# blyssprivacy/sdk

Measured on AMD Instinct MI355X. Metric: PIR queries/sec (full answer path) on 2^20 items x 256 B, higher is better.
Workload: dtype u64; 1 GPU; spiral-rs process_query, c2 = {"db_item_size": 256, "instances": 1, "n": 2, "nu_1": 9, "nu_2": 11, "p": 256, "q2_bits": 20, "t_conv": 4, "t_exp_left": 8, "t_exp_right": 56, "t_gsw": 8}, encoded DB 64.0 GiB (56.0 GiB resident per GPU), unsharded, one query per step

## Files before the change

sdk_amd/csrc/bodies.hpp:

```cpp
#pragma once
#include "device_common.hpp"

namespace spiral {

__device__ __forceinline__ void ntt_fwd_body(const DevTables& T, const FwdDesc& d, int o, int c, u32* ldsA, u32* ldsB) {
  const int tau = threadIdx.x;
  const int rows = d.rdim * d.t;
  const int per_b = rows * d.cols;
  const int b = o / per_b;
  const int rem = o - b * per_b;
  const int row = rem / d.cols, col = rem - row * d.cols;
  const int kdig = row / d.rdim, j = row - kdig * d.rdim;
  long sb = d.src_idx ? (long)d.src_idx[b] : (long)b;
  if (d.delta_off) sb = (long)(b / d.delta_inner) * d.delta_outer_stride + (b % d.delta_inner);
  const u64* src = d.src + (sb * d.src_batch_stride + (long)(d.src_row0 + j) * d.src_cols + col) * N;
  const ModConst m = T.c.mod[c];
  const int sh = kdig * d.bits;
  const bool plain = (d.bits >= 64);
  const u64 mask = plain ? ~0ULL : ((1ULL << d.bits) - 1ULL);
  u32 v[8];
#pragma unroll
  for (int k = 0; k < 8; k++) {
    u64 x = src[tau + 256 * k];
    u64 piece = (sh >= 64) ? 0ULL : ((x >> sh) & mask);
    u32 val = (d.bits <= 28) ? (u32)piece : reduce64(piece, m);
    if (d.delta_off) {
      u64 x2 = src[(size_t)d.delta_off * N + tau + 256 * k];
      u64 piece2 = (sh >= 64) ? 0ULL : ((x2 >> sh) & mask);
      u32 val2 = (d.bits <= 28) ? (u32)piece2 : reduce64(piece2, m);
      u32 a = val >= m.q ? val - m.q : val, b2 = val2 >= m.q ? val2 - m.q : val2;
      val = b2 >= a ? b2 - a : b2 + m.q - a;
    }
    v[k] = val;
  }
  const u32* fw = T.tw + (size_t)c * 4 * N;
  ntt_fwd_block(v, tau, ldsA, ldsB, fw, fw + N, m.q, m.two_q);
  uint4* dst = reinterpret_cast<uint4*>(d.dst + ((size_t)o * 2 + c) * N + 8 * tau);
  dst[0] = make_uint4(v[0], v[1], v[2], v[3]);
  dst[1] = make_uint4(v[4], v[5], v[6], v[7]);
}

__device__ __forceinline__ void ntt_inv_body(const DevTables& T, const InvDesc& d, int blk, u32* ldsA, u32* ldsB) {
  const int tau = threadIdx.x;
  int p = blk;
  long base;
  long crt_stride = d.crt_stride, z_stride = d.z_stride;
  if (d.sweep_np > 0) {
    const long np = d.sweep_np;
    if ((np % 16) == 0 && ((long)d.n_polys % 128) == 0) {
      const int b = blk;
      const int xcd = b & 7, slot = b >> 3;
      const int grp = (slot >> 4) * 8 + xcd, within = slot & 15;
      const int groups_per_plane = (int)(np / 16) * 2;
      const int plane_g = grp / groups_per_plane, rem_g = grp % groups_per_plane;
      const int r_g = rem_g / (int)(np / 16), iig = rem_g % (int)(np / 16);
      p = (int)(((long)plane_g * np + iig * 16 + within) * 2 + r_g);
    }
    const long ct = p >> 1, r = p & 1;
    const long plane = ct / np, ii = ct - plane * np;
    base = plane * 4 * N * np + r * 2 * N * np + ii;
    crt_stride = N * np;
    z_stride = np;
  } else if (d.idx) {
    int e = p / d.polys_per_idx, r = p - e * d.polys_per_idx;
    base = (long)d.idx[e] * d.idx_stride + (long)r * d.poly_stride;
  } else {
    base = (long)p * d.poly_stride;
  }
  long scal_store = -1;
  if (d.scal) {
    if (p >= d.n_polys) {
      const int e = p - d.n_polys;
      const int ct = d.scal_only_idx[e >> 1], r = e & 1;
      const long sp = ((long)(ct - d.scal_thresh) * 2 + r) * 2 * N, dp = ((long)ct * 2 + r) * 2 * N;
#pragma unroll
      for (int c = 0; c < 2; c++) {
        const uint4* a = reinterpret_cast<const uint4*>(d.src + sp + c * N + 8 * tau);
        const uint4* b = reinterpret_cast<const uint4*>(d.scal + c * N + 8 * tau);
        const uint4 a0 = a[0], a1 = a[1], b0 = b[0], b1 = b[1];
        const ModConst m = T.c.mod[c];
        uint4* o = reinterpret_cast<uint4*>(d.scal_dst + dp + c * N + 8 * tau);
        o[0] = make_uint4(reduce64((u64)a0.x * b0.x, m), reduce64((u64)a0.y * b0.y, m), reduce64((u64)a0.z * b0.z, m), reduce64((u64)a0.w * b0.w, m));
        o[1] = make_uint4(reduce64((u64)a1.x * b1.x, m), reduce64((u64)a1.y * b1.y, m), reduce64((u64)a1.z * b1.z, m), reduce64((u64)a1.w * b1.w, m));
      }
      return;
    }
    const int e = p / d.polys_per_idx, r = p - e * d.polys_per_idx;
    const int ct = d.idx[e];
    if (ct >= d.scal_thresh) {
      scal_store = base;
      base = (long)(ct - d.scal_thresh) * d.idx_stride + (long)r * d.poly_stride;
    }
  }
  u32 res[2][8];
#pragma unroll
  for (int c = 0; c < 2; c++) {
    const ModConst m = T.c.mod[c];
    const u32* src = d.src + base + (long)c * crt_stride;
    u32 v[8];
    if (z_stride == 1 && ((base | crt_stride | (scal_store < 0 ? 0 : scal_store)) & 3) == 0) {
      const uint4 a0 = reinterpret_cast<const uint4*>(src + 8 * tau)[0], a1 = reinterpret_cast<const uint4*>(src + 8 * tau)[1];
      v[0] = a0.x; v[1] = a0.y; v[2] = a0.z; v[3] = a0.w; v[4] = a1.x; v[5] = a1.y; v[6] = a1.z; v[7] = a1.w;
      if (d.premod) {
#pragma unroll
        for (int k = 0; k < 8; k++) v[k] %= m.q;
      }
      if (scal_store >= 0) {
        const uint4 s0 = reinterpret_cast<const uint4*>(d.scal + c * N + 8 * tau)[0], s1 = reinterpret_cast<const uint4*>(d.scal + c * N + 8 * tau)[1];
        const u32 sc[8] = {s0.x, s0.y, s0.z, s0.w, s1.x, s1.y, s1.z, s1.w};
#pragma unroll
        for (int k = 0; k < 8; k++) v[k] = reduce64((u64)v[k] * (u64)sc[k], m);
        uint4* o = reinterpret_cast<uint4*>(d.scal_dst + scal_store + (long)c * crt_stride + 8 * tau);
        o[0] = make_uint4(v[0], v[1], v[2], v[3]);
        o[1] = make_uint4(v[4], v[5], v[6], v[7]);
      }
    } else {
#pragma unroll
      for (int k = 0; k < 8; k++) {
        u32 x = src[(long)(8 * tau + k) * z_stride];
        if (d.premod) x = x % m.q;
        if (scal_store >= 0) {
          x = reduce64((u64)x * (u64)d.scal[c * N + 8 * tau + k], m);
          d.scal_dst[scal_store + (long)c * crt_stride + 8 * tau + k] = x;
        }
        v[k] = x;
      }
    }
    const u32* iw = inv_tables(T.tw, c);
    if (c == 1) __syncthreads();
    ntt_inv_block(v, tau, ldsA, ldsB, iw, iw + N, m.q, m.two_q);
#pragma unroll
    for (int k = 0; k < 8; k++) res[c][k] = v[k];
  }
  const u32 q0 = T.c.mod[0].q, q1 = T.c.mod[1].q;
  u64* dst = d.dst + (size_t)p * N;
#pragma unroll
  for (int k = 0; k < 8; k++) {
    u32 x = res[0][k], y = res[1][k];
    u32 xm = x >= q1 ? x - q1 : x;
    u32 dd = y >= xm ? y - xm : y + q1 - xm;
    u32 qt = __umulhi(dd, T.c.q0_inv_q1_sh);
    u32 e = dd * T.c.q0_inv_q1 - qt * q1;
    e = e >= q1 ? e - q1 : e;
    u64 val = (u64)x + (u64)q0 * (u64)e;
    int z = tau + 256 * k;
    if (d.automorph_t) {
      unsigned zt = (unsigned)z * (unsigned)d.automorph_t;
      unsigned num = zt >> POLY_LEN_LOG2, rem = zt & (N - 1);
      dst[rem] = (num & 1u) ? T.c.Q - val : val;
    } else if (d.addend) {
      const long ap = (long)(p / d.add_inner2) * d.add_outer_stride + (p % d.add_inner2);
      u64 sres = val + d.addend[(size_t)ap * N + z];
      dst[z] = sres >= T.c.Q ? sres - T.c.Q : sres;
    } else {
      dst[z] = val;
    }
  }
}

template <int CH = 28>
__device__ __forceinline__ void mac_body(const DevTables& T, const MacDesc& d, int inner, int outer, int ychunk) {
  const int e = ychunk * 256 + threadIdx.x;
  const int c = e >> POLY_LEN_LOG2;
  const int b = outer * d.batch_inner + inner;
  const ModConst m = T.c.mod[c];
  const u32* B = d.B + ((size_t)outer * d.B_outer_stride + (size_t)inner * d.B_inner_stride) * 2 * N + e;
  const long ob = d.out_idx ? (long)d.out_idx[b] : (long)b * d.out_batch_stride;
  const size_t PW = 2 * N;
  for (int r = 0; r < d.R; r++) {
    const u32* A = d.A + (size_t)r * (d.A_row_stride ? d.A_row_stride : d.K) * PW + e;
    const long op = (ob + (long)r * d.out_row_stride) * 2 * N + e;
    u64 acc = d.addend ? (u64)d.addend[op] : 0ULL;
    if (d.extra && r == d.extra_row) acc += (u64)d.extra[(size_t)(d.extra_idx ? d.extra_idx[b] : b) * PW + e];
    for (int seg = 0; seg < 2; seg++) {
      const int k_lo = seg == 0 ? 0 : d.split_k, k_hi = seg == 0 ? min(d.split_k, d.K) : d.K;
      const u32* Bs = seg == 0 ? B : B + (size_t)(d.split_off - d.split_k) * PW;
      int k = k_lo, since = 0;
      for (; k + CH <= k_hi; k += CH) {
        u32 a[CH], bb[CH];
#pragma unroll
        for (int u = 0; u < CH; u++) {
          a[u] = A[(size_t)(k + u) * PW];
          bb[u] = Bs[(size_t)(k + u) * PW];
        }
#pragma unroll
        for (int u = 0; u < CH; u++) acc += (u64)a[u] * (u64)bb[u];
        since += CH;
        if (since >= 56) {
          acc = reduce64(acc, m);
          since = 0;
        }
      }
      for (; k + 8 <= k_hi; k += 8) {
        u32 a[8], bb[8];
#pragma unroll
        for (int u = 0; u < 8; u++) {
          a[u] = A[(size_t)(k + u) * PW];
          bb[u] = Bs[(size_t)(k + u) * PW];
        }
#pragma unroll
        for (int u = 0; u < 8; u++) acc += (u64)a[u] * (u64)bb[u];
        since += 8;
        if (since >= 64) {
          acc = reduce64(acc, m);
          since = 0;
        }
      }
      for (; k < k_hi; k++) acc += (u64)A[(size_t)k * PW] * (u64)Bs[(size_t)k * PW];
      acc = reduce64(acc, m);
    }
    d.out[op] = (u32)acc;
  }
}

__device__ __forceinline__ void add_poly_into_body(const DevTables& T, u32* dst, const int* idx, const u32* src, int b, int ychunk) {
  const int e = ychunk * 256 + threadIdx.x;
  const int c = e >> POLY_LEN_LOG2;
  const long dp = (long)idx[b] * 2 * N + e;
  dst[dp] = add_mod(dst[dp], src[(size_t)b * 2 * N + e], T.c.mod[c].q);
}

__device__ __forceinline__ void copy_polys_body(const CopyPolysDesc& d, int bx, int ychunk) {
  const int e = ychunk * 256 + threadIdx.x;
  const int b = bx / d.R, r = bx % d.R;
  d.dst[((long)d.dst_idx[b] + (long)r * d.dst_row_stride) * 2 * N + e] =
      d.src[((long)d.src_idx[b] + (long)r * d.src_row_stride) * 2 * N + e];
}

__device__ __forceinline__ void folding_neg_body(const DevTables& T, const FoldingNegDesc& d, int ychunk, int by, int dd) {
  const int e = ychunk * 256 + threadIdx.x;
  const int c = e >> POLY_LEN_LOG2;
  const int col = by % d.two_t, r = by / d.two_t;
  const u32 q = T.c.mod[c].q;
  u32* row = d.mats + ((size_t)(dd * 2 + r) * 2 * d.two_t) * 2 * N;
  const u32 cv = row[(size_t)(d.two_t + col) * 2 * N + e];
  const u32 g = d.gadget_ntt[((size_t)r * d.two_t + col) * 2 * N + e];
  row[(size_t)col * 2 * N + e] = add_mod(g, cv ? q - cv : 0u, q);
}

__device__ __forceinline__ void reorient_body(const ReorientDesc& d, int bx, int by, u64* tile) {
  const int tx = threadIdx.x & 31, ty = threadIdx.x >> 5;
  const int j0 = bx * 32, z0 = by * 32;
#pragma unroll
  for (int r = 0; r < 2; r++)
#pragma unroll
    for (int i = 0; i < 4; i++) {
      const int j = j0 + ty + 8 * i;
      if (j < d.dim0) {
        const u32* p = d.v + ((size_t)(d.first + d.step * j) * 2 + r) * 2 * N;
        tile[r * (32 * 33) + (ty + 8 * i) * 33 + tx] = (u64)p[z0 + tx] | ((u64)p[N + z0 + tx] << 32);
      }
    }
  __syncthreads();
  const int w = threadIdx.x & 63, jl = w >> 1, r = w & 1, zr = threadIdx.x >> 6;
  if (j0 + jl < d.dim0) {
#pragma unroll
    for (int i = 0; i < 8; i++) {
      const int zl = zr + 4 * i;
      d.out[((size_t)(z0 + zl) * d.dim0 + j0 + jl) * 2 + r] = tile[r * (32 * 33) + jl * 33 + zl];
    }
  }
}

__host__ __device__ inline int wave_layout_word(int n) { return ((n & 31) >> 2) * 256 + (n >> 5) * 4 + (n & 3); }
__device__ __forceinline__ void mats_to_wave_body(const MatsToWaveDesc& d, size_t blk) {
  const size_t idx = blk * 256 + threadIdx.x;
  if (idx >= d.n_words) return;
  const size_t poly = idx >> POLY_LEN_LOG2;
  if (d.half_polys > 0 && (((poly >> 1) / (size_t)d.half_polys) & 1) == 0) return;
  const int n = (int)(idx & (N - 1));
  d.dst[poly * N + wave_layout_word(n)] = d.src[idx];
}

__device__ __forceinline__ u64 rescale_dev(u64 a, u64 Q, u64 out_mod) {
  u64 v = a % Q;
  const bool neg = v >= Q / 2;
  const u64 mag = neg ? Q - v : v;
  u64 lo = mag * out_mod, hi = __umul64hi(mag, out_mod);
  const u64 half = Q / 2;
  lo += half;
  hi += lo < half ? 1 : 0;
  u64 qd = (u64)(((double)hi * 18446744073709551616.0 + (double)lo) / (double)Q);
  for (int it = 0; it < 4; it++) {
    const u64 plo = qd * Q, phi = __umul64hi(qd, Q);
    const bool gt = phi > hi || (phi == hi && plo > lo);
    if (gt) {
      qd--;
      continue;
    }
    const u64 rlo = lo - plo, rhi = hi - phi - (lo < plo ? 1 : 0);
    if (rhi != 0 || rlo >= Q) {
      qd++;
      continue;
    }
    break;
  }
  const u64 base = (Q / out_mod) * out_mod + 2 * out_mod;
  const u64 r = neg ? (base - qd) % out_mod : (base + qd) % out_mod;
  return (r + out_mod) % out_mod;
}

__device__ __forceinline__ void encode_body(const EncodeDesc& d, int blk) {
  const int per_inst_first = d.n * N, per_inst_rest = d.n * d.n * N;
  const int per_inst = per_inst_first + per_inst_rest;
  const long i = (long)blk * 256 + threadIdx.x;
  if (i >= (long)d.instances * per_inst) return;
  const int inst = (int)(i / per_inst), k = (int)(i % per_inst);
  const u64* m = d.packed + (size_t)inst * (d.n + 1) * d.n * N;
  const size_t inst_bits = (size_t)per_inst_first * d.q2_bits + (size_t)per_inst_rest * d.q1_bits;
  u64 val;
  size_t bit;
  int nb;
  if (k < per_inst_first) {
    val = rescale_dev(m[k], d.Q, d.q2);
    nb = d.q2_bits;
    bit = (size_t)inst * inst_bits + (size_t)k * d.q2_bits;
  } else {
    const int kk = k - per_inst_first;
    val = rescale_dev(m[per_inst_first + kk], d.Q, d.q1);
    nb = d.q1_bits;
    bit = (size_t)inst * inst_bits + (size_t)per_inst_first * d.q2_bits + (size_t)kk * d.q1_bits;
  }
  val &= nb >= 64 ? ~0ULL : ((1ULL << nb) - 1ULL);
  const size_t w = bit >> 6;
  const int off = (int)(bit & 63);
  atomicOr(d.out + w, (unsigned long long)(val << off));
  if (off + nb > 64) atomicOr(d.out + w + 1, (unsigned long long)(val >> (64 - off)));
}

}
```

sdk_amd/csrc/elementwise.hip:

```cpp
#include "device_common.hpp"
#include "bodies.hpp"

namespace spiral {

__global__ __launch_bounds__(256) void k_mac(DevTables T, MacDesc d) { mac_body(T, d, blockIdx.x, blockIdx.z, blockIdx.y); }
__global__ __launch_bounds__(256) void k_mac2(DevTables T, MacDesc d0, MacDesc d1) {
  const int y = blockIdx.x;
  if (y < d0.batch_inner)
    mac_body(T, d0, y, 0, blockIdx.y);
  else
    mac_body(T, d1, y - d0.batch_inner, 0, blockIdx.y);
}
__global__ __launch_bounds__(256) void k_mac2_group(DevTables T, MacDesc d0, MacDesc d1, GroupOff g) {
  const int qi = blockIdx.z;
  int y = blockIdx.x;
  MacDesc d = d0;
  if (y >= d0.batch_inner) {
    d = d1;
    y -= d0.batch_inner;
  }
  d.A = group_rebase(d.A, g.pp[qi]);
  d.B = group_rebase(d.B, g.dig[qi]);
  d.out = group_rebase(d.out, g.v[qi]);
  d.addend = group_rebase(d.addend, g.v[qi]);
  d.extra = group_rebase(d.extra, g.ct1[qi]);
  mac_body(T, d, y, 0, blockIdx.y);
}
void launch_mac2_group(const DevTables& T, const MacDesc& d0, const MacDesc& d1, const GroupOff& g, int B, hipStream_t s) {
  MacDesc a = d0, b = d1;
  a.batch_inner = std::max(a.batch_inner, 0);
  b.batch_inner = std::max(b.batch_inner, 0);
  if (a.batch_inner + b.batch_inner <= 0 || B <= 0) return;
  hipLaunchKernelGGL(k_mac2_group, dim3(a.batch_inner + b.batch_inner, 2 * N / 256, B), dim3(256), 0, s, T, a, b, g);
  launched(PATH_EXPAND_GROUP, "k_mac2_group");
}
void launch_mac(const DevTables& T, const MacDesc& d, hipStream_t s) {
  if (d.batch_inner <= 0 || d.batch_outer <= 0) return;
  hipLaunchKernelGGL(k_mac, dim3(d.batch_inner, 2 * N / 256, d.batch_outer), dim3(256), 0, s, T, d);
  launched(0, "k_mac");
}
void launch_mac2(const DevTables& T, const MacDesc& d0, const MacDesc& d1, hipStream_t s) {
  MacDesc a = d0, b = d1;
  a.batch_inner = std::max(a.batch_inner, 0);
  b.batch_inner = std::max(b.batch_inner, 0);
  if (a.batch_inner + b.batch_inner <= 0) return;
  hipLaunchKernelGGL(k_mac2, dim3(a.batch_inner + b.batch_inner, 2 * N / 256, 1), dim3(256), 0, s, T, a, b);
  launched(0, "k_mac2");
}

__global__ __launch_bounds__(256) void k_add_poly_into(DevTables T, u32* dst, const int* idx, const u32* src) {
  add_poly_into_body(T, dst, idx, src, blockIdx.x, blockIdx.y);
}
void launch_add_poly_into(const DevTables& T, u32* dst, const int* idx, const u32* src, int batch, hipStream_t s) {
  if (batch <= 0) return;
  hipLaunchKernelGGL(k_add_poly_into, dim3(batch, 2 * N / 256), dim3(256), 0, s, T, dst, idx, src);
  launched(0, "k_add_poly_into");
}

__global__ __launch_bounds__(256) void k_scalar_mul(DevTables T, u32* base, long dst_off, long src_off,
                                                    const u32* scalar) {
  const int e = blockIdx.y * 256 + threadIdx.x;
  const int c = e >> POLY_LEN_LOG2;
  const long b = blockIdx.x;
  const ModConst m = T.c.mod[c];
  base[(dst_off + b) * 2 * N + e] = reduce64((u64)base[(src_off + b) * 2 * N + e] * (u64)scalar[e], m);
}
void launch_scalar_mul(const DevTables& T, u32* base, long dst_off, long src_off, const u32* scalar, int n_polys,
                       hipStream_t s) {
  if (n_polys <= 0) return;
  hipLaunchKernelGGL(k_scalar_mul, dim3(n_polys, 2 * N / 256), dim3(256), 0, s, T, base, dst_off, src_off, scalar);
  launched(0, "k_scalar_mul");
}

__global__ __launch_bounds__(256) void k_add_polys_idx(DevTables T, u32* dst, const int* di, const u32* a, const int* ai,
                                                        const u32* b, const int* bi) {
  const int e = blockIdx.y * 256 + threadIdx.x;
  const int c = e >> POLY_LEN_LOG2;
  const int k = blockIdx.x;
  dst[(size_t)di[k] * 2 * N + e] = add_mod(a[(size_t)ai[k] * 2 * N + e], b[(size_t)bi[k] * 2 * N + e], T.c.mod[c].q);
}
void launch_add_polys_idx(const DevTables& T, u32* dst, const int* di, const u32* a, const int* ai, const u32* b,
                          const int* bi, int count, hipStream_t s) {
  if (count <= 0) return;
  hipLaunchKernelGGL(k_add_polys_idx, dim3(count, 2 * N / 256), dim3(256), 0, s, T, dst, di, a, ai, b, bi);
  launched(0, "k_add_polys_idx");
}

__global__ __launch_bounds__(256) void k_interleave_query(u64* qv, const u32* row0_ntt, const u64* wire, int dim0, u32 q0,
                                                          u32 q1) {
  const size_t i = (size_t)blockIdx.x * 256 + threadIdx.x;
  if (i >= (size_t)N * dim0) return;
  const int j = (int)(i % dim0);
  const int z = (int)(i / dim0);
  const u32* p = row0_ntt + (size_t)j * 2 * N;
  qv[2 * i] = (u64)p[z] | ((u64)p[N + z] << 32);
  const u64 w = wire[i];
  qv[2 * i + 1] = (u64)((u32)w % q0) | ((u64)((u32)(w >> 32) % q1) << 32);
}
void launch_interleave_query(u64* qv, const u32* row0_ntt, const u64* wire, int dim0, hipStream_t s) {
  size_t total = (size_t)N * dim0;
  hipLaunchKernelGGL(k_interleave_query, dim3((unsigned)((total + 255) / 256)), dim3(256), 0, s, qv, row0_ntt, wire, dim0,
                     (u32)MODULUS_0, (u32)MODULUS_1);
  launched(0, "k_interleave_query");
}

__global__ __launch_bounds__(256) void k_copy_polys(CopyPolysDesc d) { copy_polys_body(d, blockIdx.x, blockIdx.y); }
void launch_copy_polys(u32* dst, const int* dst_idx, int dst_row_stride, const u32* src, const int* src_idx,
                       int src_row_stride, int R, int batch, hipStream_t s) {
  if (batch <= 0) return;
  const CopyPolysDesc d{dst, dst_idx, dst_row_stride, src, src_idx, src_row_stride, R, batch};
  hipLaunchKernelGGL(k_copy_polys, dim3(batch * R, 2 * N / 256), dim3(256), 0, s, d);
  launched(0, "k_copy_polys");
}

__global__ __launch_bounds__(256) void k_copy_polys_group(CopyPolysDesc d, GroupOff g) {
  const int qi = blockIdx.z;
  d.dst = group_rebase(d.dst, g.raw[qi]);
  d.src = group_rebase(d.src, g.v[qi]);
  copy_polys_body(d, blockIdx.x, blockIdx.y);
}
void launch_copy_polys_group(u32* dst, const int* dst_idx, int dst_row_stride, const u32* src, const int* src_idx, int src_row_stride,
                             int R, int batch, const GroupOff& g, int B, hipStream_t s) {
  if (batch <= 0 || B <= 0) return;
  const CopyPolysDesc d{dst, dst_idx, dst_row_stride, src, src_idx, src_row_stride, R, batch};
  hipLaunchKernelGGL(k_copy_polys_group, dim3(batch * R, 2 * N / 256, B), dim3(256), 0, s, d, g);
  launched(PATH_EXPAND_GROUP, "k_copy_polys_group");
}

__global__ __launch_bounds__(256) void k_checksum(const u32* p, size_t n, unsigned long long* out) {
  unsigned long long acc = 0;
  for (size_t i = (size_t)blockIdx.x * 256 + threadIdx.x; i < n; i += (size_t)gridDim.x * 256)
    acc += (unsigned long long)p[i] * (unsigned long long)((i << 1) | 1);
  atomicAdd(out, acc);
}
void launch_checksum(const u32* p, size_t n_words, unsigned long long* out, hipStream_t s) {
  hipLaunchKernelGGL(k_checksum, dim3(512), dim3(256), 0, s, p, n_words, out);
  launched(0, "k_checksum");
}
__global__ __launch_bounds__(64) void k_cache_sync(u32* sink) {
  __threadfence_system();
  if (sink && threadIdx.x == 0 && blockIdx.x == 0) sink[0] = 1;
  __threadfence_system();
}
void launch_cache_sync(u32* sink, hipStream_t s) {
  hipLaunchKernelGGL(k_cache_sync, dim3(1024), dim3(64), 0, s, sink);
  launched(0, "k_cache_sync");
}

__global__ __launch_bounds__(256) void k_copy_words(u32* dst, const u32* src, size_t n) {
  for (size_t i = (size_t)blockIdx.x * 256 + threadIdx.x; i < n; i += (size_t)gridDim.x * 256) dst[i] = src[i];
}
void launch_copy_words(u32* dst, const u32* src, size_t n_words, hipStream_t s) {
  if (n_words == 0) return;
  const unsigned blocks = (unsigned)std::min<size_t>((n_words + 255) / 256, 4096);
  hipLaunchKernelGGL(k_copy_words, dim3(blocks), dim3(256), 0, s, dst, src, n_words);
  launched(0, "k_copy_words");
}

__global__ __launch_bounds__(256) void k_folding_neg(DevTables T, FoldingNegDesc d) {
  folding_neg_body(T, d, blockIdx.x, blockIdx.y, blockIdx.z);
}
void launch_folding_neg(const DevTables& T, u32* mats, const u32* gadget_ntt, int nu2, int two_t, hipStream_t s) {
  if (nu2 <= 0) return;
  const FoldingNegDesc d{mats, gadget_ntt, two_t, nu2};
  hipLaunchKernelGGL(k_folding_neg, dim3(2 * N / 256, 2 * two_t, nu2), dim3(256), 0, s, T, d);
  launched(0, "k_folding_neg");
}

__global__ __launch_bounds__(256) void k_folding_neg_group(DevTables T, FoldingNegDesc d, GroupOff g) {
  const int qi = blockIdx.z / d.nu2;
  d.mats = group_rebase(d.mats, g.v[qi]);
  folding_neg_body(T, d, blockIdx.x, blockIdx.y, blockIdx.z - qi * d.nu2);
}
void launch_folding_neg_group(const DevTables& T, u32* mats, const u32* gadget_ntt, int nu2, int two_t, const GroupOff& g, int B,
                              hipStream_t s) {
  if (nu2 <= 0 || B <= 0) return;
  const FoldingNegDesc d{mats, gadget_ntt, two_t, nu2};
  hipLaunchKernelGGL(k_folding_neg_group, dim3(2 * N / 256, 2 * two_t, nu2 * B), dim3(256), 0, s, T, d, g);
  launched(PATH_EXPAND_GROUP, "k_folding_neg_group");
}

__global__ __launch_bounds__(256) void k_add(DevTables T, u32* out, const u32* a, const u32* b) {
  const size_t i = (size_t)blockIdx.x * 256 + threadIdx.x;
  const int c = (int)((i >> POLY_LEN_LOG2) & 1);
  out[i] = add_mod(a[i], b[i], T.c.mod[c].q);
}
void launch_add(const DevTables& T, u32* out, const u32* a, const u32* b, int n_polys, hipStream_t s) {
  if (n_polys <= 0) return;
  hipLaunchKernelGGL(k_add, dim3((unsigned)((size_t)n_polys * 2 * N / 256)), dim3(256), 0, s, T, out, a, b);
  launched(0, "k_add");
}

__global__ __launch_bounds__(256) void k_invert_raw(u64 Q, u64* out, const u64* a, long n) {
  long i = (long)blockIdx.x * 256 + threadIdx.x;
  if (i < n) out[i] = Q - a[i];
}
void launch_invert_raw(const DevTables& T, u64* out, const u64* a, long n_words, hipStream_t s) {
  if (n_words <= 0) return;
  hipLaunchKernelGGL(k_invert_raw, dim3((unsigned)((n_words + 255) / 256)), dim3(256), 0, s, T.c.Q, out, a, n_words);
  launched(0, "k_invert_raw");
}

__global__ __launch_bounds__(256) void k_automorph(u64 Q, u64* out, const u64* a, int t) {
  const int z = blockIdx.y * 256 + threadIdx.x;
  const size_t p = (size_t)blockIdx.x * N;
  unsigned zt = (unsigned)z * (unsigned)t;
  unsigned num = zt >> POLY_LEN_LOG2, rem = zt & (N - 1);
  u64 v = a[p + z];
  out[p + rem] = (num & 1u) ? Q - v : v;
}
void launch_automorph(const DevTables& T, u64* out, const u64* a, int n_polys, int t, hipStream_t s) {
  if (n_polys <= 0) return;
  hipLaunchKernelGGL(k_automorph, dim3(n_polys, N / 256), dim3(256), 0, s, T.c.Q, out, a, t);
  launched(0, "k_automorph");
}

__global__ __launch_bounds__(256) void k_gadget_raw(u64* out, const u64* inp, int cols, int rdim, int bits) {
  const int z = blockIdx.y * 256 + threadIdx.x;
  const int o = blockIdx.x;
  const int row = o / cols, col = o - row * cols;
  const int k = row / rdim, j = row - k * rdim;
  const int sh = k * bits;
  const u64 mask = bits >= 64 ? ~0ULL : ((1ULL << bits) - 1ULL);
  u64 x = inp[((size_t)j * cols + col) * N + z];
  out[(size_t)o * N + z] = sh >= 64 ? 0ULL : ((x >> sh) & mask);
}
void launch_gadget_raw(u64* out, const u64* inp, int rows_in, int cols, int rows_out, int rdim, int bits,
                       hipStream_t s) {
  (void)rows_in;
  hipLaunchKernelGGL(k_gadget_raw, dim3(rows_out * cols, N / 256), dim3(256), 0, s, out, inp, cols, rdim, bits);
  launched(0, "k_gadget_raw");
}

__global__ __launch_bounds__(256) void k_u64_to_u32(u32* out, const u64* in, long n) {
  long i = (long)blockIdx.x * 256 + threadIdx.x;
  if (i < n) out[i] = (u32)in[i];
}
__global__ __launch_bounds__(256) void k_u32_to_u64(u64* out, const u32* in, long n) {
  long i = (long)blockIdx.x * 256 + threadIdx.x;
  if (i < n) out[i] = (u64)in[i];
}
void launch_u64_to_u32(u32* out, const u64* in, long n, hipStream_t s) {
  if (n <= 0) return;
  hipLaunchKernelGGL(k_u64_to_u32, dim3((unsigned)((n + 255) / 256)), dim3(256), 0, s, out, in, n);
  launched(0, "k_u64_to_u32");
}
void launch_u32_to_u64(u64* out, const u32* in, long n, hipStream_t s) {
  if (n <= 0) return;
  hipLaunchKernelGGL(k_u32_to_u64, dim3((unsigned)((n + 255) / 256)), dim3(256), 0, s, out, in, n);
  launched(0, "k_u32_to_u64");
}

__global__ __launch_bounds__(256) void k_encode(EncodeDesc d) { encode_body(d, blockIdx.x); }
void launch_encode(const EncodeDesc& d, hipStream_t s) {
  const long total = (long)d.instances * ((long)d.n * N + (long)d.n * d.n * N);
  hipLaunchKernelGGL(k_encode, dim3((unsigned)((total + 255) / 256)), dim3(256), 0, s, d);
  launched(0, "k_encode");
}

__global__ __launch_bounds__(256) void k_reorient(ReorientDesc d) {
  __shared__ u64 tile[2 * 32 * 33];
  reorient_body(d, blockIdx.x, blockIdx.y, tile);
}
void launch_reorient(u64* out, const u32* v, int first, int step, int dim0, hipStream_t s) {
  const ReorientDesc d{out, v, first, step, dim0};
  hipLaunchKernelGGL(k_reorient, dim3((dim0 + 31) / 32, N / 32), dim3(256), 0, s, d);
  launched(0, "k_reorient");
}

__global__ __launch_bounds__(256) void k_reorient_group(ReorientDesc d, GroupOff g) {
  __shared__ u64 tile[2 * 32 * 33];
  const int qi = blockIdx.z;
  d.out = group_rebase(d.out, g.raw[qi]);
  d.v = group_rebase(d.v, g.v[qi]);
  reorient_body(d, blockIdx.x, blockIdx.y, tile);
}
void launch_reorient_group(u64* out, const u32* v, int first, int step, int dim0, const GroupOff& g, int B, hipStream_t s) {
  if (B <= 0) return;
  const ReorientDesc d{out, v, first, step, dim0};
  hipLaunchKernelGGL(k_reorient_group, dim3((dim0 + 31) / 32, N / 32, B), dim3(256), 0, s, d, g);
  launched(PATH_EXPAND_GROUP, "k_reorient_group");
}

__global__ __launch_bounds__(64) void k_cu_probe(u32* out) {
  u32 xcc, hw;
  asm volatile("s_getreg_b32 %0, hwreg(HW_REG_XCC_ID)" : "=s"(xcc));
  asm volatile("s_getreg_b32 %0, hwreg(HW_REG_HW_ID)" : "=s"(hw));
  u32 acc = threadIdx.x;
  for (int i = 0; i < 20000; i++) acc = acc * 1664525u + 1013904223u;
  if (threadIdx.x == 0) {
    out[blockIdx.x * 2] = xcc;
    out[blockIdx.x * 2 + 1] = hw | ((acc & 1u) << 31);
  }
}
void launch_cu_probe(u32* out, int blocks, hipStream_t s) {
  hipLaunchKernelGGL(k_cu_probe, dim3(blocks), dim3(64), 0, s, out);
  launched(0, "k_cu_probe");
}

}

#include "pp_raw_image.hpp"
```

sdk_amd/csrc/kernels.hpp:

```cpp
#pragma once
#include <hip/hip_runtime.h>

#include <vector>

#include "params.hpp"

namespace spiral {

constexpr int N = (int)POLY_LEN;

struct DevTables {
  const u32* tw;
  DevConsts c;
};
__host__ __device__ inline const u32* inv_tables(const u32* tw, int c) { return tw + (size_t)8 * N + (size_t)c * 2 * N; }
__host__ __device__ inline const u32* wave_fwd_image(const u32* tw, int c) { return tw + (size_t)12 * N + (size_t)c * 2 * N; }
__host__ __device__ inline int wtw_phys(int idx) {
  if (idx >= 1024) {
    const int L = (idx - 1024) >> 4, r = (idx - 1024) & 15;
    return 1024 + 16 * L + 4 * (((r >> 2) + (L >> 2)) & 3) + (r & 3);
  }
  if (idx >= 512) {
    const int L = (idx - 512) >> 3, r = (idx - 512) & 7;
    return 512 + 8 * L + 4 * (((r >> 2) + (L >> 3)) & 1) + (r & 3);
  }
  return idx;
}

enum PathBit : u64 {
  PATH_SWEEP_PERSIST = 1ull << 0,
  PATH_SWEEP_PACKED = 1ull << 1,
  PATH_SWEEP_WIDE = 1ull << 2,
  PATH_SWEEP_NARROW = 1ull << 3,
  PATH_SWEEP_BATCH = 1ull << 4,
  PATH_FROM_SWEEP4 = 1ull << 5,
  PATH_FROM_SWEEP1 = 1ull << 6,
  PATH_FOLD_FUSED = 1ull << 7,
  PATH_FOLD_TAIL = 1ull << 8,
  PATH_FOLD_TAIL_LITERAL = 1ull << 9,
  PATH_PIPELINED = 1ull << 10,
  PATH_EXPAND_PRUNED = 1ull << 11,
  PATH_PACK_V1 = 1ull << 12,
  PATH_DIRECT_UPLOAD = 1ull << 13,
  PATH_SCATTER_OUT = 1ull << 14,
  PATH_SWEEP_XCD_FROM = 1ull << 15,
  PATH_FOLD_TAIL_PERSIST = 1ull << 16,
  PATH_EXPAND_FUSED = 1ull << 17,
  PATH_SWEEP_SPARSE = 1ull << 18,
  PATH_RCCL = 1ull << 19,
  PATH_FOLD_WAVE = 1ull << 20,
  PATH_CU_SPLIT = 1ull << 21,
  PATH_EXPAND_SPLIT = 1ull << 22,
  PATH_PIPE_CLASS_SPLIT = 1ull << 23,
  PATH_SWEEP_MFMA = 1ull << 24,
  PATH_CUSTOM_TRANSPORT = 1ull << 25,
  PATH_FROM_SWEEP_WAVE = 1ull << 26,
  PATH_FOLD_TAIL_BATCHED = 1ull << 27,
  PATH_SWEEP_RING = 1ull << 28,
  PATH_SWEEP_MFMA2 = 1ull << 29,
  PATH_FOLD_WAVE8 = 1ull << 30,
  PATH_SWEEP_PLANAR = 1ull << 31,
  PATH_EXPAND_GROUP = 1ull << 32,
  PATH_EXPAND_WAVE = 1ull << 33,
  PATH_SWEEP_BATCH_SCATTER = 1ull << 34,
  PATH_SWEEP_SPARSE_GROUP = 1ull << 35,
  PATH_SWEEP_NARROW_GROUP = 1ull << 36
};
long tunable(const char* name, long dflt);
void launched(u64 path_bits, const char* kernel);
void note_path(u64 path_bits);
void launch_checksum(const u32* p, size_t n_words, unsigned long long* out, hipStream_t s);
void launch_cache_sync(u32* sink, hipStream_t s);
void launch_copy_words(u32* dst, const u32* src, size_t n_words, hipStream_t s);
void debug_stage(int stage);

struct FwdDesc {
  const u64* src;
  const int* src_idx;
  u32* dst;
  int n_out;
  int rdim, cols, t, bits;
  int src_batch_stride;
  int src_row0, src_cols;
  long delta_off;
  int delta_inner, delta_outer_stride;
};
void launch_ntt_fwd(const DevTables& T, const FwdDesc& d, hipStream_t s);
void launch_ntt_fwd3(const DevTables& T, const FwdDesc& d0, const FwdDesc& d1, const FwdDesc& d2, hipStream_t s);

float bench_ntt_core(const DevTables& T, int M, int blocks, int reps, u32* scratch, hipStream_t s);

struct InvDesc {
  const u32* src;
  const int* idx;
  int polys_per_idx;
  long idx_stride, poly_stride, crt_stride, z_stride;
  u64* dst;
  int n_polys;
  int premod;
  int sweep_np;
  int automorph_t;
  const u32* scal;
  u32* scal_dst;
  int scal_thresh;
  const int* scal_only_idx;
  int n_scalar_only;
  const u64* addend;
  int add_inner2, add_outer_stride;
};
void launch_ntt_inv(const DevTables& T, const InvDesc& d, hipStream_t s);
void launch_from_sweep4(const DevTables& T, const u32* src, int np, int n_planes, int premod, u64* dst, hipStream_t s);

struct MacDesc {
  const u32* A;
  const u32* B;
  u32* out;
  const u32* addend;
  const int* out_idx;
  int R, K;
  int A_row_stride;
  int batch_inner, batch_outer;
  long B_inner_stride, B_outer_stride;
  int split_k;
  long split_off;
  int out_batch_stride, out_row_stride;
  const u32* extra;
  const int* extra_idx;
  int extra_row;
};
void launch_mac(const DevTables& T, const MacDesc& d, hipStream_t s);
void launch_mac2(const DevTables& T, const MacDesc& d0, const MacDesc& d1, hipStream_t s);

struct ExpandSideDesc {
  const u64* raw;
  const int* pos;
  const int* out_idx;
  const u32* A;
  u32* v;
  int cnt, t, bits;
};
void launch_expand_round(const DevTables& T, const ExpandSideDesc& left, const ExpandSideDesc& right, hipStream_t s);
constexpr long EXPAND_ROUND_MIN_DEFAULT = 2048;

constexpr int GROUP_MAX = 16;
struct GroupOff {
  long long v[GROUP_MAX], raw[GROUP_MAX], dig[GROUP_MAX], ct1[GROUP_MAX], pp[GROUP_MAX];
};
void launch_ntt_inv_group(const DevTables& T, const InvDesc& d, const GroupOff& g, int B, hipStream_t s);
void launch_ntt_fwd3_group(const DevTables& T, const FwdDesc& d0, const FwdDesc& d1, const FwdDesc& d2, const GroupOff& g, int B,
                           hipStream_t s);
void launch_mac2_group(const DevTables& T, const MacDesc& d0, const MacDesc& d1, const GroupOff& g, int B, hipStream_t s);
void launch_expand_round_group(const DevTables& T, const ExpandSideDesc& left, const ExpandSideDesc& right, const GroupOff& g, int B,
                               hipStream_t s);
void launch_reorient_group(u64* out, const u32* v, int first, int step, int dim0, const GroupOff& g, int B, hipStream_t s);
void launch_copy_polys_group(u32* dst, const int* dst_idx, int dst_row_stride, const u32* src, const int* src_idx, int src_row_stride,
                             int R, int batch, const GroupOff& g, int B, hipStream_t s);
void launch_folding_neg_group(const DevTables& T, u32* mats, const u32* gadget_ntt, int nu2, int two_t, const GroupOff& g, int B,
                              hipStream_t s);
void launch_mats_to_wave_group(u32* dst, const u32* src, size_t n_words, int half_polys, const GroupOff& g, int B, hipStream_t s);
struct ExpandWaveDesc {
  const u64* raw;
  const int* pos;
  const int* out_idx;
  const u32* A_w;
  const u32* const_w;
  u32* v;
  int cnt, t, bits;
};
void launch_expand_wave(const DevTables& T, const ExpandWaveDesc& d, const GroupOff& g, int B, hipStream_t s);
constexpr long EXPAND_WAVE_MIN_DIGITS_DEFAULT = 16;
constexpr long EXPAND_GROUP_ROUND_MIN_DEFAULT = 4096;

struct FoldDesc {
  const u64* X;
  u64* Y;
  const u32* mats;
  int cur, half, planes;
  int t, bits;
  int t_live;
  int zero_shortcuts;
  const u32* mats_w;
};
void launch_mats_to_wave(u32* dst, const u32* src, size_t n_words, hipStream_t s, int half_polys = 0);
constexpr long FOLD_VARIANT_DEFAULT = 5;
void launch_fold_fused(const DevTables& T, const FoldDesc& d, hipStream_t s);

void launch_add_poly_into(const DevTables& T, u32* dst, const int* idx, const u32* src, int batch, hipStream_t s);
void launch_scalar_mul(const DevTables& T, u32* base, long dst_off, long src_off, const u32* scalar, int n_polys,
                       hipStream_t s);
void launch_add_polys_idx(const DevTables& T, u32* dst, const int* di, const u32* a, const int* ai, const u32* b,
                          const int* bi, int count, hipStream_t s);
void launch_interleave_query(u64* qv, const u32* row0_ntt, const u64* wire, int dim0, hipStream_t s);
void launch_copy_polys(u32* dst, const int* dst_idx, int dst_row_stride, const u32* src, const int* src_idx,
                       int src_row_stride, int R, int batch, hipStream_t s);
void launch_folding_neg(const DevTables& T, u32* mats, const u32* gadget_ntt, int nu2, int two_t, hipStream_t s);
void launch_add(const DevTables& T, u32* out, const u32* a, const u32* b, int n_polys, hipStream_t s);
void launch_invert_raw(const DevTables& T, u64* out, const u64* a, long n_words, hipStream_t s);
void launch_automorph(const DevTables& T, u64* out, const u64* a, int n_polys, int t, hipStream_t s);
void launch_gadget_raw(u64* out, const u64* inp, int rows_in, int cols, int rows_out, int rdim, int bits,
                       hipStream_t s);
void launch_u64_to_u32(u32* out, const u64* in, long n, hipStream_t s);
void launch_u32_to_u64(u64* out, const u32* in, long n, hipStream_t s);

void launch_cu_probe(u32* out, int blocks, hipStream_t s);

struct EncodeDesc {
  const u64* packed;
  unsigned long long* out;
  int instances, n;
  u64 Q, q1, q2;
  int q1_bits, q2_bits;
};
void launch_encode(const EncodeDesc& d, hipStream_t s);

void launch_reorient(u64* out, const u32* v, int first, int step, int dim0, hipStream_t s);

struct CopyPolysDesc {
  u32* dst;
  const int* dst_idx;
  int dst_row_stride;
  const u32* src;
  const int* src_idx;
  int src_row_stride, R, batch;
};
struct FoldingNegDesc {
  u32* mats;
  const u32* gadget_ntt;
  int two_t, nu2;
};
struct ReorientDesc {
  u64* out;
  const u32* v;
  int first, step, dim0;
};
struct MatsToWaveDesc {
  u32* dst;
  const u32* src;
  size_t n_words;
  int half_polys;
};
struct AddPolyIntoDesc {
  u32* dst;
  const int* idx;
  const u32* src;
  int batch;
};
struct CopyWordsDesc {
  u32* dst;
  const u32* src;
  size_t n_words;
};
constexpr u64 PP_RAW_WIRE = 1ull << 63;
struct PpRawDesc {
  u64* dst;
  const u64* wire;
  const u64* table;
  u64 n_words;
  u64 modulus, modulus_inv;
};
void launch_pp_raw_image(const PpRawDesc& d, int n_polys, hipStream_t s);

struct SweepDesc {
  const u64* db;
  const u64* qv;
  u32* out;
  int planes, num_per, dim0, j0, nj;
  int packed;
  int out_G;
  int nt_store;
};
struct ColMap {
  int off = 0, stride = 1, np_global = 0;
};
inline bool db_can_pack(int num_per, int nj) { return num_per >= 128 && (nj % 2) == 0; }
inline size_t db_bytes(int planes, int num_per, int nj, bool packed) {
  return (size_t)planes * N * nj * num_per * (packed ? 7 : 8);
}
void launch_sweep(const DevTables& T, const SweepDesc& d, hipStream_t s);
void launch_sweep_persist(const DevTables& T, const SweepDesc& d, int wgs_per_cu, hipStream_t s, int n_cus = 256);
constexpr int SWEEP_BATCH_MAX = 8;
constexpr int SWEEP_GROUP_MAX = 16;
struct SweepBatchDesc {
  const u64* db;
  const u64* qv[SWEEP_GROUP_MAX];
  u32* out[SWEEP_GROUP_MAX];
  int batch;
  int planes, num_per, dim0, j0, nj;
  u32* rq;
  int use_mfma;
  const unsigned char* planar;
  int narrow;
  int fold_every;
};
bool sweep_narrow_batch_shape_ok(int num_per, int nj);
constexpr long NARROW_BATCH_MIN_DEFAULT = 0;
void launch_sweep_narrow_batch(const DevTables& T, const SweepBatchDesc& d, hipStream_t s);
bool sweep_planar_shape_ok(int num_per, int nj);
size_t sweep_planar_bytes(int planes, int num_per, int nj);
void launch_packed_to_planar(unsigned char* planar, const u64* packed, int planes, int num_per, int nj, hipStream_t s);
void launch_planar_patch_item(unsigned char* planar, const u64* packed, int planes, int num_per, int nj, int j, int ii, hipStream_t s);
constexpr size_t UPSERT_MAX_GROUP_PLANES = (size_t)1 << 23;
struct PlanarPatchCell {
  int j, ii;
};
void launch_planar_patch_items(unsigned char* planar, const u64* packed, int planes, int num_per, int nj, const PlanarPatchCell* cells,
                               size_t n_cells, hipStream_t s);
void launch_sweep_planar(const DevTables& T, const SweepBatchDesc& d, hipStream_t s);
bool planar_resident_shape_ok(int num_per, int nj);
int planar_resident_group_max(int nj);
struct PlanarShardShape {
  int dim0 = 0;
  int j0 = 0;
  int G = 1;
};
void launch_planar_from_ref(unsigned char* planar, const u64* src, int plane, int z0, int nz, int num_per, int nj, PlanarShardShape sh,
                            hipStream_t s);
void launch_planar_synth(unsigned char* planar, u64 seed, int planes, int num_per, int nj, PlanarShardShape sh, hipStream_t s);
void launch_planar_from_stage(unsigned char* planar, const u64* stage, int planes, int jg, int ii0, int ncols, int num_per, int nj,
                              PlanarShardShape sh, hipStream_t s);
void launch_planar_put_items(unsigned char* planar, const u64* stage, int planes, size_t np_s, const PlanarPatchCell* cells, size_t n_items,
                             int num_per, int nj, PlanarShardShape sh, hipStream_t s);
void launch_planar_read(u64* out, const unsigned char* planar, int plane, int z, int ii, int jl0, int count, int num_per, int nj,
                        PlanarShardShape sh, hipStream_t s);
void sweep_planar_resident_prepare(const DevTables& T, SweepBatchDesc& d, hipStream_t s);
void launch_sweep_planar_resident(const DevTables& T, const SweepBatchDesc& d, hipStream_t s);
void launch_sweep_planar_scatter(const DevTables& T, const SweepBatchDesc& d, int G, int plane0, int total_planes, bool all_planes,
                                 hipStream_t s);
bool sweep_batch_wants_mfma(const SweepBatchDesc& d);
int sweep_batch_group_max(int num_per, int nj);
inline int sweep_batch_tiles(int batch) { return batch > SWEEP_BATCH_MAX ? 2 : 1; }
inline size_t sweep_batch_rq_words(int nj, int tiles = 1) {
  return (size_t)tiles * ((size_t)N * (size_t)(nj / 16) * 128 * 4 + (size_t)N * 32);
}
void sweep_batch_prepare(const DevTables& T, SweepBatchDesc& d, hipStream_t s);
void launch_sweep_batch(const DevTables& T, const SweepBatchDesc& d, hipStream_t s);
constexpr long BATCH_SCATTER_STORE_DEFAULT = 2;
constexpr long BATCH_SCATTER_MAX_G_DEFAULT = 8;
bool sweep_batch_scatter_ok(const SweepBatchDesc& d, int G);
void launch_sweep_batch_scatter(const DevTables& T, const SweepBatchDesc& d, int G, hipStream_t s);
void launch_db_relayout(u64* dst, int plane, const u64* src, int z0, int nz, int num_per, int dim0, int j0, int nj,
                        int packed, ColMap cm, hipStream_t s);
void launch_canon_words(u64* w, size_t total, hipStream_t s);
void launch_db_synth(u64* dst, u64 seed, int planes, int num_per, int dim0, int j0, int nj, int packed, ColMap cm,
                     hipStream_t s);
void launch_db_read(u64* out, const u64* db, int plane, int z, int ii, int jl0, int count, int num_per, int nj,
                    int packed, hipStream_t s);
struct DbEncodeDesc {
  const uint8_t* win;
  size_t win_item0;
  size_t win_bytes;
  size_t file_len;
  u64* db;
  int db_item_size, bytes_per_chunk, logp;
  u32 pt_modulus;
  int planes, num_per, dim0, j0, nj, packed;
  int jp0, njp;
  long only_item;
  int only_q;
  ColMap cm;
};
void launch_db_encode(const DevTables& T, const DbEncodeDesc& d, hipStream_t s);
struct DbQuadRec {
  int jp, q;
  int len[4];
  long long src[4];
};
void launch_db_encode_quads(const DevTables& T, const DbEncodeDesc& d, const DbQuadRec* quads, size_t n_quads, hipStream_t s);

void launch_items_gather(u64* dst, const u64* db, size_t L0, size_t nL, int np_local, int nj, int planes, int packed, hipStream_t s);
void launch_planar_gather(u64* dst, const unsigned char* planar, size_t L0, size_t nL, int num_per, int nj, int planes, PlanarShardShape sh,
                          hipStream_t s);
struct ItemDecodeRec {
  int src, pos;
};
struct ItemDecodeDesc {
  const u64* src;
  const ItemDecodeRec* list;
  uint8_t* out;
  unsigned long long* undecodable;
  int planes, db_item_size, bytes_per_chunk, logp;
  u32 pt_modulus;
};
void launch_items_decode(const DevTables& T, const ItemDecodeDesc& d, size_t n_items, hipStream_t s);

void launch_items_scatter_words8(u64* db, const u64* stage, const int* src_of, size_t D0, size_t nD, int np_local, int nj, int planes,
                                 hipStream_t s);
struct CopyQuadRec {
  int jp, q;
  int src[4];
};
void launch_items_scatter_packed(u64* db, const u64* stage, const CopyQuadRec* quads, size_t n_quads, int np_local, int nj, int planes,
                                 hipStream_t s);
struct CopyCellRec {
  int j, ii;
  int src[16];
};
void launch_planar_scatter_items(unsigned char* planar, const u64* stage, const CopyCellRec* cells, size_t n_cells, int num_per, int nj,
                                 int planes, PlanarShardShape sh, hipStream_t s);
struct CopySlotRec {
  int src, slot;
};
void launch_items_copy_slots(u64* polys, const u64* stage, const CopySlotRec* recs, size_t n_recs, int planes, hipStream_t s);

void launch_sparse_item_encode(const DevTables& T, const uint8_t* bytes, int item_bytes, int bytes_per_chunk, int logp,
                               u32 pt_modulus, u64* slot_polys, int planes, hipStream_t s);
struct SparseItemRec {
  unsigned long long off;
  int len, slot;
};
void launch_sparse_items_encode(const DevTables& T, const uint8_t* win, const SparseItemRec* items, size_t n_items, int item_bytes,
                                int bytes_per_chunk, int logp, u32 pt_modulus, u64* polys, int planes, hipStream_t s);
void launch_sweep_sparse(const DevTables& T, const int* col_ptr, const int* col_rows, const int* col_slots, const u64* polys,
                         int planes, const u32* v, int first, int step, u32* out, int num_per, hipStream_t s);
constexpr int SPARSE_GROUP_MAX = 8;
constexpr long SPARSE_BATCH_MIN_DEFAULT = 2;
struct SparseGroup {
  const u32* v[SPARSE_GROUP_MAX];
  u32* out[SPARSE_GROUP_MAX];
};
void launch_sweep_sparse_batch(const DevTables& T, const int* col_ptr, const int* col_rows, const int* col_slots, const u64* polys,
                               int planes, const SparseGroup& members, int nq, int first, int step, int num_per, hipStream_t s);
void launch_sweep_sparse_scatter(const DevTables& T, const int* col_ptr, const int* col_rows, const int* col_slots, const u64* polys,
                                 int planes, int plane0, int n_planes, const u32* v, int first, int step, u32* out, int num_per, int G,
                                 bool per_plane, hipStream_t s);
void launch_sweep_sparse_scatter_batch(const DevTables& T, const int* col_ptr, const int* col_rows, const int* col_slots, const u64* polys,
                                       int planes, const SparseGroup& members, int nq, int first, int step, int num_per, int G,
                                       hipStream_t s);

void launch_sweep_out_to_ref(u64* out, const u32* in, int num_per, hipStream_t s);

__host__ __device__ inline u64 synth_word(u64 seed, u64 idx) {
  u64 z = seed + 0x9E3779B97F4A7C15ULL * (idx + 1);
  z = (z ^ (z >> 30)) * 0xBF58476D1CE4E5B9ULL;
  z = (z ^ (z >> 27)) * 0x94D049BB133111EBULL;
  z ^= z >> 31;
  u64 lo = (u32)z % (u32)MODULUS_0;
  u64 hi = (u32)(z >> 32) % (u32)MODULUS_1;
  return lo | (hi << 32);
}

__host__ __device__ inline u64 digest_mix(u64 x) {
  x += 0x9E3779B97F4A7C15ULL;
  x = (x ^ (x >> 30)) * 0xBF58476D1CE4E5B9ULL;
  x = (x ^ (x >> 27)) * 0x94D049BB133111EBULL;
  return x ^ (x >> 31);
}
__host__ __device__ inline u64 digest_col_key(u64 s, u64 c) { return digest_mix(s ^ c) | 1ULL; }
__host__ __device__ inline u64 digest_row_key(u64 s, u64 j) { return digest_mix(~s ^ j) | 1ULL; }
constexpr int DIGEST_ROWS = 1024;
struct DigestDesc {
  unsigned long long* sums;
  const u64* R;
  u64 s[2];
  int plane0, nplanes;
  int num_per;
  int nj;
};
void launch_digest_keys(unsigned long long* sums, u64* R, u64 seed, int nplanes, int j0, int nj, hipStream_t s);
void launch_digest_words(const DigestDesc& d, const u64* db, int np_local, int packed, ColMap cm, hipStream_t s);
struct DigestSlotRec {
  unsigned long long slot, item;
};
void launch_digest_sparse(const DigestDesc& d, const u64* polys, int planes, const DigestSlotRec* list, size_t n, hipStream_t s);
void launch_digest_planar(const DigestDesc& d, const unsigned char* planar, PlanarShardShape sh, hipStream_t s);

constexpr int ITEM_DIGEST_Z = 64;
struct ItemDigestDesc {
  unsigned long long* table;
  const u64* R;
  u64 s[2];
  int plane0, nplanes;
  int num_per;
  int nj;
  int jl0, nrows;
};
void launch_item_digest_words(const ItemDigestDesc& d, const u64* db, int np_local, int packed, ColMap cm, hipStream_t s);
void launch_item_digest_sparse(const ItemDigestDesc& d, const u64* polys, int planes, const DigestSlotRec* list, size_t n,
                               unsigned long long item_base, uint8_t* present, hipStream_t s);
void launch_item_digest_planar(const ItemDigestDesc& d, const unsigned char* planar, PlanarShardShape sh, hipStream_t s);

}
```

sdk_amd/csrc/pipeline.hpp:

```cpp
#pragma once
#include <vector>

#include "server.hpp"

namespace spiral {

struct Workspace {
  const Params* P;
  DeviceState* D;
  int device = -1;
  hipStream_t stream = nullptr;
  hipStream_t stream2 = nullptr;
  std::vector<hipEvent_t> ev_plane;
  hipEvent_t ev_fold = nullptr;
  hipEvent_t ev_round0 = nullptr, ev_right = nullptr;
  bool right_pending = false;
  bool long_sweep_follows = false;
  hipEvent_t ev_sw[2] = {nullptr, nullptr};
  bool have_sweep_span = false;
  bool pipelined = false;
  hipEvent_t ev[5] = {nullptr, nullptr, nullptr, nullptr, nullptr};
  DevBuf<u64> q_raw;
  DevBuf<u32> v;
  DevBuf<u64> exp_raw;
  DevBuf<u32> exp_dig;
  DevBuf<u32> exp_ct1;
  DevBuf<u64> exp_raw_r;
  DevBuf<u32> exp_dig_r, exp_ct1_r;
  DevBuf<u64> qv;
  DevBuf<u32> fold_mats;
  DevBuf<u32> fold_mats_w;
  bool mats_w_ready = false;
  DevBuf<u64> gsw_raw;
  DevBuf<u32> gsw_dig;
  DevBuf<u32> sweep_out;
  DevBuf<u64> fold_tail;
  DevBuf<u32> batch_rq;
  DevBuf<u64> foldX, foldY, final_cts, pack_raw;
  DevBuf<u32> fold_dig, fold_ntt, pack_dig, pack_ct2, pack_res, pack_v1_P, pack_v1_P2;
  DevBuf<u64> pack_v1_raw, du_raw, du_wire;
  DevBuf<u32> du_ntt;
  u64* h_query = nullptr;
  u64* h_group_query = nullptr;
  DevBuf<u64> group_q_raw;
  u64* h_packed = nullptr;
  size_t h_packed_words = 0;
  DevBuf<u64> enc_out;
  uint8_t* h_response = nullptr;
  bool host_pinned = true;
  int out_G = 1;
  bool zero_shortcuts = false;
  long fused_min_pairs = 256;

  Workspace(const Params& P, DeviceState& D);
  ~Workspace();
  Workspace(const Workspace&) = delete;
  Workspace& operator=(const Workspace&) = delete;
  void ensure_expand();
  void ensure_sweep();
  void ensure_finish();
  size_t plane_group() const;
};

void run_coefficient_expansion(Workspace& W, const sp_pp& pp, size_t g_rounds, const DeviceState::PrunedPlan* plan = nullptr,
                               int tree = 0, size_t r_begin = 0);
void join_right(Workspace& W);
void run_regev_to_gsw(Workspace& W, const sp_pp& pp, const u32* v_src, const int* src_ct, const int* src_poly);
void run_folding_neg(Workspace& W);
void run_mats_to_wave(Workspace& W, size_t levels, bool c_only = false);
void run_fold_operands(Workspace& W);
void run_begin_direct(Workspace& W, const uint8_t* query);
void run_begin_group(Workspace* const* Ws, const sp_pp* const* pps, const uint8_t* const* queries, const size_t* query_lens, int B);
void run_begin(Workspace& W, const sp_pp& pp, const uint8_t* query, size_t query_len, int j0 = 0, int nj = 0,
               const DeviceState::PrunedPlan* plan = nullptr);
void run_sweep_sparse(Workspace& W, const sp_db& db, const int* col_ptr, const int* col_rows, const int* col_slots);
void run_sweep_sparse_group(Workspace* const* Ws, int B, const sp_db& db, const int* col_ptr, const int* col_rows, const int* col_slots,
                            hipStream_t s);
void run_sweep_sparse_scatter(Workspace& W, const sp_db& db, const int* col_ptr, const int* col_rows, const int* col_slots, int G,
                              int plane0, int n_planes, bool per_plane);
void run_sweep_sparse_scatter_group(Workspace* const* Ws, int B, const sp_db& db, const int* col_ptr, const int* col_rows,
                                    const int* col_slots, int G, hipStream_t s);
std::unique_ptr<DeviceState::PrunedPlan> build_pruned_plan_rows(const Params& P, const std::vector<char>& rows);
void run_sweep(Workspace& W, const sp_db& db);
void run_sweep_pipelined(Workspace& W, const sp_db& db);
bool sweep_is_pipelined(const Params& p, const sp_db& db);
void launch_plane_sweep(Workspace& W, const sp_db& db, size_t plane);
bool fused_fold_supported(const Params& p);
struct FoldOpts {
  long fused_min_pairs;
  bool delta_tail;
  bool inputs_below_q;
};
u64* run_fold(Workspace& W, const FoldOpts& o, u64* X, u64* Y, int np, int num_cts, int top, int d_begin = 0, int d_end = -1);
void run_fold_local(Workspace& W, const u32* reduced_chunk, int G);
void run_fold_local_plane(Workspace& W, const u32* reduced_plane_chunk, int G, int plane);
void run_fold_local_join(Workspace& W);
void run_finish_gathered(Workspace& W, const sp_pp& pp, const u64* gathered, int G);
void run_fold_all(Workspace& W, bool premod);
void run_pack(Workspace& W, const sp_pp& pp);
void run_finish(Workspace& W, const sp_pp& pp, bool premod);
size_t encode_response(const Params& p, const u64* packed, uint8_t* out);
void run_encode_device(Workspace& W);

}
```

sdk_amd/csrc/server.cpp:

```cpp
#include "server.hpp"

#include <algorithm>
#include <atomic>
#include <cstdlib>
#include <cstring>
#include <functional>

#include "pipeline.hpp"

namespace spiral {

void hip_check(hipError_t e, const char* what, const char* file, int line) {
  if (e != hipSuccess) {
    (void)hipGetLastError();
    throw HipError(std::string(what) + " failed at " + file + ":" + std::to_string(line) + ": " + hipGetErrorString(e));
  }
}

static std::mutex g_tun_mu;
static std::vector<std::pair<std::string, long>> g_tun;
static std::atomic<unsigned> g_tun_epoch{1};
static std::atomic<long> g_fresh_allocs{0};
void tunables_new_call() { g_tun_epoch.fetch_add(1, std::memory_order_relaxed); }
void set_tunable(const char* name, long v) {
  if (!strcmp(name, "poison_skip")) g_fresh_allocs = 0;
  {
    std::lock_guard<std::mutex> lk(g_tun_mu);
    bool found = false;
    for (auto& kv : g_tun)
      if (kv.first == name) {
        kv.second = v;
        found = true;
        break;
      }
    if (!found) g_tun.emplace_back(name, v);
  }
  tunables_new_call();
}
static bool tunable_resolve(const char* name, long* out) {
  {
    std::lock_guard<std::mutex> lk(g_tun_mu);
    for (auto& kv : g_tun)
      if (kv.first == name) {
        *out = kv.second;
        return true;
      }
  }
  std::string env = "SPIRAL_";
  for (const char* c = name; *c; c++) env += (char)toupper((unsigned char)*c);
  const char* e = getenv(env.c_str());
  if (!e) return false;
  *out = atol(e);
  return true;
}
long tunable(const char* name, long dflt) {
  struct Ent {
    std::string name;
    unsigned epoch;
    bool has;
    long val;
  };
  thread_local std::vector<Ent> cache;
  const unsigned ep = g_tun_epoch.load(std::memory_order_relaxed);
  for (auto& e : cache)
    if (!strcmp(e.name.c_str(), name)) {
      if (e.epoch != ep) {
        e.has = tunable_resolve(name, &e.val);
        e.epoch = ep;
      }
      return e.has ? e.val : dflt;
    }
  Ent e{name, ep, false, 0};
  e.has = tunable_resolve(name, &e.val);
  cache.push_back(e);
  return e.has ? e.val : dflt;
}

void devbuf_fresh(void* p, size_t bytes) {
  const long b = tunable("poison_ws", 0);
  if (b <= 0 || !p || tunable("guard_ws", 0) > 0) return;
  const long k = g_fresh_allocs.fetch_add(1);
  const bool skip = tunable("poison_skip", -1) == k;
  if (getenv("SPIRAL_ALLOC_DEBUG")) fprintf(stderr, "[spiral] alloc #%ld: %zu bytes%s\n", k, bytes, skip ? " (zeroed)" : "");
  HIP_CHECK(hipMemset(p, skip ? 0 : (int)(b & 255), bytes));
  HIP_CHECK(hipDeviceSynchronize());
}
void devbuf_cache_sync();
bool devbuf_guards_on() { return tunable("guard_ws", 0) > 0; }
void* devbuf_alloc(size_t bytes, size_t* guard, long* serial) {
  const long g = tunable("guard_ws", 0);
  const size_t gb = g > 0 ? ((size_t)g + 255) / 256 * 256 : 0;
  void* q = nullptr;
  const hipError_t e = hipMalloc(&q, bytes + 2 * gb);
  if (e != hipSuccess) {
    (void)hipGetLastError();
    throw OomError(std::string("hipMalloc of ") + std::to_string(bytes) + " bytes failed: " + hipGetErrorString(e));
  }
  *guard = gb;
  *serial = -1;
  if (getenv("SPIRAL_ALLOC_DEBUG")) fprintf(stderr, "[spiral] hipMalloc %zu bytes -> [%p, %p)\n", bytes + 2 * gb, q, (char*)q + bytes + 2 * gb);
  void* const block = q;
  try {
  if (gb) {
    const long k = g_fresh_allocs.fetch_add(1);
    *serial = k;
    const bool skip = tunable("poison_skip", -1) == k;
    const int fill = skip ? 0 : (int)(tunable("poison_ws", 0xA5) & 255);
    if (getenv("SPIRAL_ALLOC_DEBUG")) fprintf(stderr, "[spiral] alloc #%ld: %zu bytes%s\n", k, bytes, skip ? " (guards zeroed)" : "");
    HIP_CHECK(hipMemset(q, fill, gb));
    HIP_CHECK(hipMemset((char*)q + gb + bytes, fill, gb));
    HIP_CHECK(hipDeviceSynchronize());
    q = (char*)q + gb;
  }
  devbuf_fresh(q, bytes);
  if (!gb && tunable("poison_ws", 0) <= 0 && tunable("alloc_zero", 1) != 0) {
    HIP_CHECK(hipMemset(q, 0, bytes));
    devbuf_cache_sync();
    HIP_CHECK(hipDeviceSynchronize());
  }
  } catch (...) {
    (void)hipFree(block);
    throw;
  }
  return q;
}
void devbuf_cache_sync() {
  if (tunable("alloc_cache_sync", 0) != 0) launch_cache_sync(nullptr, 0);
}
void devbuf_free(void* p, size_t bytes, size_t guard, long serial) {
  if (!p) return;
  if (getenv("SPIRAL_ALLOC_DEBUG")) fprintf(stderr, "[spiral] hipFree %p\n", (void*)((char*)p - guard));
  if (guard) {
    (void)hipDeviceSynchronize();
    std::vector<unsigned char> h(2 * guard);
    if (hipMemcpy(h.data(), (char*)p - guard, guard, hipMemcpyDeviceToHost) == hipSuccess &&
        hipMemcpy(h.data() + guard, (char*)p + bytes, guard, hipMemcpyDeviceToHost) == hipSuccess) {
      long first_before = -1, last_after = -1;
      for (size_t i = 0; i < guard; i++)
        if (h[i] != h[0]) { first_before = (long)(guard - i); break; }
      for (size_t i = 0; i < guard; i++)
        if (h[guard + i] != h[2 * guard - 1]) last_after = (long)i;
      if (first_before >= 0 || last_after >= 0)
        fprintf(stderr, "[spiral] OUT-OF-BOUNDS WRITE around alloc #%ld (%zu bytes): reaches %ld bytes before / %ld bytes after\n",
                serial, bytes, first_before, last_after);
    }
    (void)hipGetLastError();
  }
  (void)hipFree((char*)p - guard);
}

extern thread_local int g_debug_stage;
void h2d_sync(void* dst, const void* host, size_t bytes) {
  if (bytes == 0) return;
  HIP_CHECK(hipMemcpy(dst, host, bytes, hipMemcpyHostToDevice));
  if (tunable("h2d_cache_sync", 0) != 0) launch_cache_sync(nullptr, 0);
}
void upload_words(void* dst, const void* host, size_t bytes) {
  h2d_sync(dst, host, bytes);
  HIP_CHECK(hipDeviceSynchronize());
}

static thread_local u64 g_paths = 0;
void note_path(u64 bits) { g_paths |= bits; }
u64 paths_taken(bool reset) {
  const u64 v = g_paths;
  if (reset) g_paths = 0;
  return v;
}
void launched(u64 bits, const char* kernel) {
  g_paths |= bits;
  const hipError_t e = hipGetLastError();
  if (e != hipSuccess) throw HipError(std::string("launch of ") + kernel + " failed: " + hipGetErrorString(e));
  const long ds = tunable("debug_sync", 0);
  if (ds == 1 || (ds > 10 && ds == 10 + g_debug_stage)) HIP_CHECK(hipDeviceSynchronize());
}
thread_local int g_debug_stage = 0;
void debug_stage(int stage) {
  g_debug_stage = stage;
  if (tunable("debug_sync", 0) == 2) HIP_CHECK(hipDeviceSynchronize());
}

static inline u32 rotl(u32 v, int c) { return (v << c) | (v >> (32 - c)); }
static inline void quarter(u32* s, int a, int b, int c, int d) {
  s[a] += s[b]; s[d] = rotl(s[d] ^ s[a], 16);
  s[c] += s[d]; s[b] = rotl(s[b] ^ s[c], 12);
  s[a] += s[b]; s[d] = rotl(s[d] ^ s[a], 8);
  s[c] += s[d]; s[b] = rotl(s[b] ^ s[c], 7);
}
static void chacha_block(const u32 init[16], u64 ctr, u32 out[16]) {
  u32 in0[16], s[16];
  memcpy(in0, init, sizeof(in0));
  in0[12] = (u32)ctr;
  in0[13] = (u32)(ctr >> 32);
  in0[14] = in0[15] = 0;
  memcpy(s, in0, sizeof(s));
  for (int rnd = 0; rnd < 10; rnd++) {
    quarter(s, 0, 4, 8, 12); quarter(s, 1, 5, 9, 13); quarter(s, 2, 6, 10, 14); quarter(s, 3, 7, 11, 15);
    quarter(s, 0, 5, 10, 15); quarter(s, 1, 6, 11, 12); quarter(s, 2, 7, 8, 13); quarter(s, 3, 4, 9, 14);
  }
  for (int i = 0; i < 16; i++) out[i] = s[i] + in0[i];
}
#if defined(__x86_64__)
}
#include <immintrin.h>
namespace spiral {
__attribute__((target("avx2"))) static void chacha_blocks8_avx2(const u32 init[16], u64 ctr0, u32 (*out)[16]) {
  __m256i in0[16], s[16];
  for (int i = 0; i < 16; i++) in0[i] = _mm256_set1_epi32((int)init[i]);
  alignas(32) u32 lo[8], hi[8];
  for (int l = 0; l < 8; l++) {
    const u64 c = ctr0 + (u64)l;
    lo[l] = (u32)c;
    hi[l] = (u32)(c >> 32);
  }
  in0[12] = _mm256_load_si256(reinterpret_cast<const __m256i*>(lo));
  in0[13] = _mm256_load_si256(reinterpret_cast<const __m256i*>(hi));
  in0[14] = in0[15] = _mm256_setzero_si256();
  for (int i = 0; i < 16; i++) s[i] = in0[i];
#define SP_ROT(x, n) _mm256_or_si256(_mm256_slli_epi32(x, n), _mm256_srli_epi32(x, 32 - n))
#define SP_QR(a, b, c, d)                                                                              \
  s[a] = _mm256_add_epi32(s[a], s[b]); s[d] = _mm256_xor_si256(s[d], s[a]); s[d] = SP_ROT(s[d], 16);   \
  s[c] = _mm256_add_epi32(s[c], s[d]); s[b] = _mm256_xor_si256(s[b], s[c]); s[b] = SP_ROT(s[b], 12);   \
  s[a] = _mm256_add_epi32(s[a], s[b]); s[d] = _mm256_xor_si256(s[d], s[a]); s[d] = SP_ROT(s[d], 8);    \
  s[c] = _mm256_add_epi32(s[c], s[d]); s[b] = _mm256_xor_si256(s[b], s[c]); s[b] = SP_ROT(s[b], 7);
  for (int rnd = 0; rnd < 10; rnd++) {
    SP_QR(0, 4, 8, 12) SP_QR(1, 5, 9, 13) SP_QR(2, 6, 10, 14) SP_QR(3, 7, 11, 15)
    SP_QR(0, 5, 10, 15) SP_QR(1, 6, 11, 12) SP_QR(2, 7, 8, 13) SP_QR(3, 4, 9, 14)
  }
#undef SP_QR
#undef SP_ROT
  alignas(32) u32 tmp[16][8];
  for (int i = 0; i < 16; i++) _mm256_store_si256(reinterpret_cast<__m256i*>(tmp[i]), _mm256_add_epi32(s[i], in0[i]));
  for (int l = 0; l < 8; l++)
    for (int i = 0; i < 16; i++) out[l][i] = tmp[i][l];
}
static bool cpu_has_avx2() { return __builtin_cpu_supports("avx2"); }
#else
static void chacha_blocks8_avx2(const u32*, u64, u32 (*)[16]) {}
static bool cpu_has_avx2() { return false; }
#endif

void chacha20_keystream_u64(const uint8_t seed[32], u64* out, size_t count) {
  u32 init[16] = {0x61707865u, 0x3320646eu, 0x79622d32u, 0x6b206574u};
  for (int i = 0; i < 8; i++) {
    u32 w;
    memcpy(&w, seed + 4 * i, 4);
    init[4 + i] = w;
  }
  static const bool avx2 = cpu_has_avx2();
  const bool wide = avx2 && tunable("chacha_scalar", 0) == 0;
  u64 ctr = 0;
  size_t done = 0;
  u32 blk[8][16];
  while (done < count) {
    int have = 1;
    if (wide && count - done >= 16) {
      chacha_blocks8_avx2(init, ctr, blk);
      have = 8;
    } else {
      chacha_block(init, ctr, blk[0]);
    }
    ctr += (u64)have;
    for (int l = 0; l < have && done < count; l++)
      for (int i = 0; i < 16 && done < count; i += 2, done++) out[done] = (u64)blk[l][i] | ((u64)blk[l][i + 1] << 32);
  }
}

struct FastMod {
  u64 Q, m;
  explicit FastMod(u64 q) : Q(q), m(q > 1 ? (u64)(((unsigned __int128)1 << 64) / q) : 0) {}
  u64 operator()(u64 x) const {
    u64 r = x - (u64)(((unsigned __int128)x * m) >> 64) * Q;
    while (r >= Q) r -= Q;
    return r;
  }
};

static std::vector<RoundPlan> build_round_plans(const Params& P, int j0, int nj, std::vector<int>& L,
                                                const std::vector<char>* row_set = nullptr, int side = 0) {
  auto put = [&](const std::vector<int>& v) {
    size_t off = L.size();
    L.insert(L.end(), v.begin(), v.end());
    return off;
  };
  std::vector<RoundPlan> rounds;
  const size_t g = P.g();
  const size_t nu2 = P.db_dim_2;
  const size_t stop_round = nu2 > 0 ? P.stop_round() : 0;
  const size_t max_bits_right = nu2 > 0 ? P.t_gsw * nu2 : 0;
  const bool prune = nu2 > 0 && (row_set != nullptr || j0 != 0 || nj != (int)P.dim0());
  for (size_t r = 0; r < g; r++) {
    RoundPlan rp;
    rp.num_in = 1 << r;
    rp.t_auto = (int)(POLY_LEN >> r) + 1;
    std::vector<char> need_even((size_t)2 << r, 1);
    if (prune) {
      std::fill(need_even.begin(), need_even.end(), 0);
      const size_t mod = (size_t)2 << r;
      if (row_set) {
        for (size_t j = 0; j < row_set->size(); j++)
          if ((*row_set)[j]) need_even[((size_t)2 * j) % mod] = 1;
      } else if ((size_t)nj * 2 >= mod) {
        std::fill(need_even.begin(), need_even.end(), 1);
      } else {
        for (int j = j0; j < j0 + nj; j++) need_even[((size_t)2 * j) % mod] = 1;
      }
    }
    std::vector<int> all_ct, all_row1, lpos, lout, rpos, rout, skip2, lct, rct;
    for (int half = 0; half < 2; half++)
      for (int i = 0; i < rp.num_in; i++) {
        bool skip = (stop_round > 0 && r > stop_round && (i % 2) == 1) ||
                    (stop_round > 0 && r == stop_round && (i % 2) == 1 && (size_t)(i / 2) >= max_bits_right);
        const int ct = half * rp.num_in + i;
        const bool even_tree = r != 0 && (i % 2) == 0;
        if ((side == 1 && !even_tree) || (side == 2 && even_tree)) continue;
        if (skip) {
          if (half == 1 && !prune) skip2.push_back(rp.num_in + i);
          continue;
        }
        if (r != 0 && (i % 2) == 0 && !need_even[ct]) continue;
        int pos = (int)all_ct.size();
        all_ct.push_back(ct);
        all_row1.push_back(ct * 2 + 1);
        if (r != 0 && (i % 2) == 0) {
          lpos.push_back(pos);
          lout.push_back(ct * 2);
          lct.push_back(ct);
        } else {
          rpos.push_back(pos);
          rout.push_back(ct * 2);
          rct.push_back(ct);
        }
      }
    rp.n_all = (int)all_ct.size();
    rp.n_left = (int)lpos.size();
    rp.n_right = (int)rpos.size();
    rp.all_ct = put(all_ct);
    rp.all_row1 = put(all_row1);
    rp.left_pos = put(lpos);
    rp.left_out = put(lout);
    rp.right_pos = put(rpos);
    rp.right_out = put(rout);
    rp.left_ct = put(lct);
    rp.right_ct = put(rct);
    rp.skip2 = put(skip2);
    rp.n_skip2 = (int)skip2.size();
    rounds.push_back(rp);
  }
  return rounds;
}

const DeviceState::PrunedPlan& DeviceState::pruned_plan(const Params& P, int j0, int nj) {
  std::lock_guard<std::mutex> lk(pruned_mu);
  for (auto& pp : pruned)
    if (pp->j0 == j0 && pp->nj == nj) return *pp;
  auto pl = std::make_unique<PrunedPlan>();
  pl->j0 = j0;
  pl->nj = nj;
  std::vector<int> L;
  pl->rounds = build_round_plans(P, j0, nj, L);
  pl->rounds_even = build_round_plans(P, j0, nj, L, nullptr, 1);
  pl->rounds_odd = build_round_plans(P, j0, nj, L, nullptr, 2);
  pl->lists.alloc(std::max<size_t>(L.size(), 1));
  if (!L.empty()) upload_words(pl->lists.p, L.data(), L.size() * sizeof(int));
  pruned.push_back(std::move(pl));
  return *pruned.back();
}

std::unique_ptr<DeviceState::PrunedPlan> build_pruned_plan_rows(const Params& P, const std::vector<char>& rows) {
  auto pl = std::make_unique<DeviceState::PrunedPlan>();
  pl->j0 = -1;
  pl->nj = -1;
  std::vector<int> L;
  pl->rounds = build_round_plans(P, 0, 0, L, &rows);
  pl->rounds_even = build_round_plans(P, 0, 0, L, &rows, 1);
  pl->rounds_odd = build_round_plans(P, 0, 0, L, &rows, 2);
  pl->lists.alloc(std::max<size_t>(L.size(), 1));
  if (!L.empty()) upload_words(pl->lists.p, L.data(), L.size() * sizeof(int));
  return pl;
}

static std::unique_ptr<DeviceState> build_device_state(const Params& P, int device) {
  auto D = std::make_unique<DeviceState>();
  D->device = device;
  D->tw.alloc(P.ntt_tables.size());
  upload_words(D->tw.p, P.ntt_tables.data(), P.ntt_tables.size() * sizeof(u32));
  D->T.tw = D->tw.p;
  D->T.c = P.dc;
  const size_t g = P.expand_queries ? P.g() : 0;
  const size_t nu2 = P.db_dim_2;

  {
    std::vector<u64> raw(std::max<size_t>(g, 1) * POLY_LEN, 0);
    for (size_t r = 0; r < g && r < POLY_LEN_LOG2; r++) raw[r * POLY_LEN + (POLY_LEN - ((size_t)1 << r))] = P.modulus - 1;
    DevBuf<u64> d_raw(raw.size());
    h2d_sync(d_raw.p, raw.data(), raw.size() * 8);
    D->neg1.alloc(std::max<size_t>(g, 1) * 2 * POLY_LEN);
    FwdDesc f{d_raw.p, nullptr, D->neg1.p, (int)g, 1, 1, 1, 64, 1, 0, 1};
    launch_ntt_fwd(D->T, f, 0);
    HIP_CHECK(hipDeviceSynchronize());
  }
  {
    const size_t cols = 2 * P.t_gsw, bits = P.bits_per(P.t_gsw);
    std::vector<u64> raw(2 * cols * POLY_LEN, 0);
    for (size_t i = 0; i < 2; i++)
      for (size_t j = 0; j < P.t_gsw; j++) {
        if (bits * j >= 64) continue;
        raw[(i * cols + (i + j * 2)) * POLY_LEN] = 1ULL << (bits * j);
      }
    DevBuf<u64> d_raw(raw.size());
    h2d_sync(d_raw.p, raw.data(), raw.size() * 8);
    D->gadget_gsw.alloc(2 * cols * 2 * POLY_LEN);
    FwdDesc f{d_raw.p, nullptr, D->gadget_gsw.p, (int)(2 * cols), 1, 1, 1, 64, 1, 0, 1};
    launch_ntt_fwd(D->T, f, 0);
    HIP_CHECK(hipDeviceSynchronize());
  }

  std::vector<int> L;
  auto put = [&](const std::vector<int>& v) {
    size_t off = L.size();
    L.insert(L.end(), v.begin(), v.end());
    return off;
  };
  if (P.expand_queries) {
    D->rounds = build_round_plans(P, 0, (int)P.dim0(), L);
    D->rounds_even = build_round_plans(P, 0, (int)P.dim0(), L, nullptr, 1);
    D->rounds_odd = build_round_plans(P, 0, (int)P.dim0(), L, nullptr, 2);
    for (const RoundPlan& rp : D->rounds) {
      D->max_all = std::max(D->max_all, (size_t)rp.n_all);
      D->max_left = std::max(D->max_left, (size_t)rp.n_left);
      D->max_right = std::max(D->max_right, (size_t)rp.n_right);
    }
  }
  {
    std::vector<int> src_ct, src_poly, out_even, out_odd;
    for (size_t d = 0; d < nu2; d++)
      for (size_t j = 0; j < P.t_gsw; j++) {
        int b = (int)(d * P.t_gsw + j);
        src_ct.push_back(2 * b + 1);
        src_poly.push_back((2 * b + 1) * 2);
        int row0 = (int)(d * 2 * 4 * P.t_gsw + 2 * P.t_gsw);
        out_even.push_back(row0 + (int)(2 * j));
        out_odd.push_back(row0 + (int)(2 * j + 1));
      }
    D->gsw_src_ct = put(src_ct);
    D->gsw_src_poly = put(src_poly);
    D->gsw_out_even = put(out_even);
    D->gsw_out_odd = put(out_odd);
  }
  {
    std::vector<int> src_ct, out, row;
    const int n = (int)P.n;
    for (int inst = 0; inst < (int)P.instances; inst++)
      for (int c = 0; c < n; c++) {
        out.push_back(inst * (n + 1) * n + c);
        for (int r = 0; r < n; r++) {
          src_ct.push_back(inst * n * n + r * n + c);
          row.push_back(inst * (n + 1) * n + (1 + r) * n + c);
        }
      }
    D->pack_src_ct = put(src_ct);
    D->pack_out = put(out);
    D->pack_row = put(row);
  }
  if (P.version == 1 && P.n == 2) {
    std::vector<int> row1, ssrc, rd, ra, rb, sd, sa, sb;
    const int ne = (int)P.instances * 2;
    for (int b = 0; b < ne * 2; b++) row1.push_back(b * 3 + 1);
    for (int e = 0; e < ne; e++) {
      const int inst = e / 2, c = e % 2, b0 = e * 2, b1 = e * 2 + 1;
      ssrc.push_back(b1 * 3);
      rd.push_back(e * 3 + 1); ra.push_back(e * 3 + 1); rb.push_back(b1 * 3 + 2);
      rd.push_back(e * 3 + 2); ra.push_back(e * 3 + 2); rb.push_back(b1 * 3 + 1);
      for (int rr = 0; rr < 3; rr++) {
        sd.push_back(inst * 6 + rr * 2 + c);
        sa.push_back(b0 * 3 + rr);
        sb.push_back(e * 3 + rr);
      }
    }
    D->v1_row1 = put(row1);
    D->v1_shift_src = put(ssrc);
    D->v1_rot_dst = put(rd); D->v1_rot_a = put(ra); D->v1_rot_b = put(rb);
    D->v1_sum_dst = put(sd); D->v1_sum_a = put(sa); D->v1_sum_b = put(sb);
  }
  D->lists.alloc(std::max<size_t>(L.size(), 1));
  if (!L.empty()) upload_words(D->lists.p, L.data(), L.size() * sizeof(int));
  return D;
}

}

using namespace spiral;

DeviceState& sp_params::device_state() {
  int dev = 0;
  HIP_CHECK(hipGetDevice(&dev));
  std::lock_guard<std::mutex> lk(mu);
  for (auto& d : this->dev)
    if (d->device == dev) return *d;
  this->dev.push_back(build_device_state(p, dev));
  return *this->dev.back();
}

std::unique_ptr<Workspace> sp_params::acquire_ws() {
  int dev = 0;
  HIP_CHECK(hipGetDevice(&dev));
  {
    std::lock_guard<std::mutex> lk(mu);
    for (size_t i = 0; i < ws_pool.size(); i++)
      if (ws_pool[i]->device == dev) {
        auto w = std::move(ws_pool[i]);
        ws_pool.erase(ws_pool.begin() + i);
        return w;
      }
  }
  auto w = std::make_unique<Workspace>(p, device_state());
  if (tunable("ws_prealloc", 1) != 0) {
    if (p.expand_queries) w->ensure_expand();
    w->ensure_sweep();
    w->ensure_finish();
    HIP_CHECK(hipDeviceSynchronize());
  }
  return w;
}

void sp_params::release_ws(std::unique_ptr<Workspace> ws) {
  std::lock_guard<std::mutex> lk(mu);
  ws_pool.push_back(std::move(ws));
}

sp_params::~sp_params() {}

namespace spiral {

static int tail_defer_levels(const Params& p, long stop);
Workspace::Workspace(const Params& P, DeviceState& D) : P(&P), D(&D) {
  device = D.device;
  HIP_CHECK(hipStreamCreateWithFlags(&stream, hipStreamNonBlocking));
  HIP_CHECK(hipStreamCreateWithFlags(&stream2, hipStreamNonBlocking));
  HIP_CHECK(hipEventCreateWithFlags(&ev_fold, hipEventDisableTiming));
  HIP_CHECK(hipEventCreateWithFlags(&ev_round0, hipEventDisableTiming));
  HIP_CHECK(hipEventCreateWithFlags(&ev_right, hipEventDisableTiming));
  ev_plane.resize(P.planes());
  for (auto& e : ev_plane) HIP_CHECK(hipEventCreateWithFlags(&e, hipEventDisableTiming));
  for (auto& e : ev) HIP_CHECK(hipEventCreate(&e));
  for (auto& e : ev_sw) HIP_CHECK(hipEventCreate(&e));
  h_packed_words = P.instances * (P.n + 1) * P.n * POLY_LEN;
  host_pinned = tunable("ws_pinned", 1) != 0;
  if (host_pinned) {
    HIP_CHECK(hipHostMalloc((void**)&h_query, 2 * POLY_LEN * sizeof(u64), hipHostMallocDefault));
    HIP_CHECK(hipHostMalloc((void**)&h_packed, h_packed_words * sizeof(u64), hipHostMallocDefault));
    HIP_CHECK(hipHostMalloc((void**)&h_response, P.response_bytes() + 16, hipHostMallocDefault));
  } else {
    h_query = (u64*)malloc(2 * POLY_LEN * sizeof(u64));
    h_packed = (u64*)malloc(h_packed_words * sizeof(u64));
    h_response = (uint8_t*)malloc(P.response_bytes() + 16);
    if (!h_query || !h_packed || !h_response) throw OomError("host staging allocation failed");
  }
  enc_out.alloc(P.response_bytes() / 8 + 2);
  q_raw.alloc(2 * POLY_LEN);
  fused_min_pairs = tunable("fused_min_pairs", 256);
}

Workspace::~Workspace() {
  if (host_pinned) {
    if (h_query) (void)hipHostFree(h_query);
    if (h_group_query) (void)hipHostFree(h_group_query);
    if (h_packed) (void)hipHostFree(h_packed);
    if (h_response) (void)hipHostFree(h_response);
  } else {
    free(h_query);
    free(h_group_query);
    free(h_packed);
    free(h_response);
  }
  for (auto& e : ev)
    if (e) (void)hipEventDestroy(e);
  for (auto& e : ev_plane)
    if (e) (void)hipEventDestroy(e);
  if (ev_fold) (void)hipEventDestroy(ev_fold);
  for (hipEvent_t e : {ev_sw[0], ev_sw[1], ev_round0, ev_right})
    if (e) (void)hipEventDestroy(e);
  if (stream2) (void)hipStreamDestroy(stream2);
  if (stream) (void)hipStreamDestroy(stream);
}

void Workspace::ensure_expand() {
  const Params& p = *P;
  const size_t g = p.g();
  v.ensure(((size_t)1 << g) * 2 * 2 * POLY_LEN);
  exp_raw.ensure(std::max<size_t>(D->max_all, 1) * 2 * POLY_LEN);
  size_t dig = D->max_left * p.t_exp_left + D->max_right * p.t_exp_right;
  exp_dig.ensure(std::max<size_t>(dig, 1) * 2 * POLY_LEN);
  exp_ct1.ensure(std::max<size_t>(D->max_all, 1) * 2 * POLY_LEN);
  if (p.db_dim_2 > 0) {
    exp_raw_r.ensure(std::max<size_t>(D->max_all, 1) * 2 * POLY_LEN);
    exp_dig_r.ensure(std::max<size_t>(D->max_right * p.t_exp_right, 1) * 2 * POLY_LEN);
    exp_ct1_r.ensure(std::max<size_t>(D->max_all, 1) * 2 * POLY_LEN);
  }
  qv.ensure(POLY_LEN * p.dim0() * 2);
  const size_t nb = p.db_dim_2 * p.t_gsw;
  fold_mats.ensure(std::max<size_t>(p.db_dim_2, 1) * 2 * 4 * p.t_gsw * 2 * POLY_LEN);
  if (p.db_dim_2 > 0 && fused_fold_supported(p)) fold_mats_w.ensure(p.db_dim_2 * 2 * 4 * p.t_gsw * 2 * POLY_LEN);
  gsw_raw.ensure(std::max<size_t>(nb, 1) * 2 * POLY_LEN);
  gsw_dig.ensure(std::max<size_t>(nb, 1) * 2 * p.t_conv * 2 * POLY_LEN);
}

size_t Workspace::plane_group() const {
  const Params& p = *P;
  const bool fused_ok = fused_fold_supported(p) && fused_min_pairs < (1L << 40);
  size_t per_plane = p.num_per() * 2 * POLY_LEN * sizeof(u64) * 2;
  if (!fused_ok) per_plane += p.num_per() * 2 * p.t_gsw * 2 * POLY_LEN * sizeof(u32);
  size_t budget = (size_t)2 << 30;
  size_t pg = std::max<size_t>(1, budget / std::max<size_t>(per_plane, 1));
  return std::min(pg, p.planes());
}

void Workspace::ensure_sweep() {
  const Params& p = *P;
  sweep_out.ensure(p.planes() * 4 * POLY_LEN * p.num_per());
}

void Workspace::ensure_finish() {
  const Params& p = *P;
  const size_t pg = plane_group();
  foldX.ensure(pg * p.num_per() * 2 * POLY_LEN);
  foldY.ensure(std::max<size_t>(pg * p.num_per() / 2, 1) * 2 * POLY_LEN);
  const bool fused_ok = fused_fold_supported(p);
  size_t dig_cts = pg * p.num_per();
  if (fused_ok && fused_min_pairs < (1L << 40)) dig_cts = std::min<size_t>(dig_cts, std::max<size_t>(2 * (size_t)fused_min_pairs, 2 * pg));
  fold_dig.ensure(dig_cts * 2 * p.t_gsw * 2 * POLY_LEN);
  fold_ntt.ensure(std::max<size_t>(dig_cts / 2, 1) * 2 * 2 * POLY_LEN);
  final_cts.ensure(p.planes() * 2 * POLY_LEN);
  const size_t nb = p.planes();
  pack_dig.ensure(nb * p.t_conv * 2 * POLY_LEN);
  pack_ct2.ensure(nb * 2 * POLY_LEN);
  pack_res.ensure(p.instances * (p.n + 1) * p.n * 2 * POLY_LEN);
  pack_raw.ensure(p.instances * (p.n + 1) * p.n * POLY_LEN);
  const int defer = tail_defer_levels(p, tunable("pipe_tail_defer", 256));
  if (defer > 0 && p.num_per() >= 1024) fold_tail.ensure(2 * p.planes() * (p.num_per() >> defer) * 2 * POLY_LEN);
}

static void on_stream(Workspace& W, hipStream_t s, const std::function<void()>& f) {
  hipStream_t saved = W.stream;
  W.stream = s;
  try {
    f();
  } catch (...) {
    W.stream = saved;
    throw;
  }
  W.stream = saved;
}

void join_right(Workspace& W);

struct RoundLaunches {
  InvDesc inv;
  FwdDesc fd[3];
  MacDesc md[2];
  ExpandSideDesc es[2];
  long round_transforms;
  bool digits_fit;
};
static RoundLaunches round_launches(Workspace& W, const sp_pp& pp, const RoundPlan& rp, size_t r, const int* L, int tree) {
  const Params& p = *W.P;
  DeviceState& D = *W.D;
  u64* const exp_raw = tree == 2 ? W.exp_raw_r.p : W.exp_raw.p;
  u32* const exp_dig = tree == 2 ? W.exp_dig_r.p : W.exp_dig.p;
  u32* const exp_ct1 = tree == 2 ? W.exp_ct1_r.p : W.exp_ct1.p;
  const int tl = (int)p.t_exp_left, tr = (int)p.t_exp_right;
  RoundLaunches R{};
  InvDesc& inv = R.inv;
  inv.src = W.v.p;
  inv.idx = L + rp.all_ct;
  inv.polys_per_idx = 2;
  inv.idx_stride = 4 * POLY_LEN;
  inv.poly_stride = 2 * POLY_LEN;
  inv.crt_stride = POLY_LEN;
  inv.z_stride = 1;
  inv.dst = exp_raw;
  inv.n_polys = rp.n_all * 2;
  inv.automorph_t = rp.t_auto;
  inv.scal = D.neg1.p + r * 2 * POLY_LEN;
  inv.scal_dst = W.v.p;
  inv.scal_thresh = rp.num_in;
  inv.scal_only_idx = L + rp.skip2;
  inv.n_scalar_only = rp.n_skip2;
  for (int side = 0; side < 2; side++) {
    const int cnt = side == 0 ? rp.n_left : rp.n_right;
    const int t = side == 0 ? tl : tr;
    FwdDesc f{};
    f.src = exp_raw;
    f.src_idx = L + (side == 0 ? rp.left_pos : rp.right_pos);
    f.dst = exp_dig + (side == 0 ? 0 : (size_t)rp.n_left * tl * 2 * POLY_LEN);
    f.n_out = cnt * t;
    f.rdim = 1;
    f.cols = 1;
    f.t = t;
    f.bits = (int)p.bits_per(t);
    f.src_batch_stride = 2;
    f.src_row0 = 0;
    f.src_cols = 1;
    R.fd[side] = f;
  }
  {
    FwdDesc f1{};
    f1.src = exp_raw;
    f1.dst = exp_ct1;
    f1.n_out = rp.n_all;
    f1.rdim = 1;
    f1.cols = 1;
    f1.t = 1;
    f1.bits = 64;
    f1.src_batch_stride = 2;
    f1.src_row0 = 1;
    f1.src_cols = 1;
    R.fd[2] = f1;
  }
  R.round_transforms = (long)rp.n_left * tl + (long)rp.n_right * tr;
  R.digits_fit = R.fd[0].bits <= 28 && R.fd[1].bits <= 28;
  for (int side = 0; side < 2; side++) {
    const int cnt = side == 0 ? rp.n_left : rp.n_right;
    const int t = side == 0 ? tl : tr;
    const bool use_right = side == 1 && pp.has_right && p.db_dim_2 > 0;
    const size_t woff = use_right ? pp.off_right + r * 2 * tr : pp.off_left + r * 2 * tl;
    MacDesc m{};
    m.A = pp.all.p + woff * 2 * POLY_LEN;
    m.B = R.fd[side].dst;
    m.out = W.v.p;
    m.addend = W.v.p;
    m.out_idx = L + (side == 0 ? rp.left_out : rp.right_out);
    m.R = 2;
    m.K = t;
    m.batch_inner = cnt;
    m.batch_outer = 1;
    m.B_inner_stride = t;
    m.B_outer_stride = 0;
    m.split_k = t;
    m.split_off = 0;
    m.out_batch_stride = 0;
    m.out_row_stride = 1;
    m.extra = exp_ct1;
    m.extra_idx = L + (side == 0 ? rp.left_pos : rp.right_pos);
    m.extra_row = 1;
    R.md[side] = m;
    R.es[side] = ExpandSideDesc{R.fd[side].src, R.fd[side].src_idx, m.out_idx, m.A, m.out, m.batch_inner, R.fd[side].t, R.fd[side].bits};
  }
  return R;
}

void run_coefficient_expansion(Workspace& W, const sp_pp& pp, size_t g_rounds, const DeviceState::PrunedPlan* plan,
                               int tree, size_t r_begin) {
  DeviceState& D = *W.D;
  hipStream_t s = W.stream;
  const int* L = plan ? plan->lists.p : D.lists.p;
  const std::vector<RoundPlan>& rounds = tree == 1   ? (plan ? plan->rounds_even : D.rounds_even)
                                         : tree == 2 ? (plan ? plan->rounds_odd : D.rounds_odd)
                                                     : (plan ? plan->rounds : D.rounds);
  for (size_t r = r_begin; r < g_rounds; r++) {
    const RoundPlan& rp = rounds[r];
    if (rp.n_all == 0 && (tree != 0 || rp.n_skip2 == 0)) continue;
    const RoundLaunches R = round_launches(W, pp, rp, r, L, tree);
    const bool one_launch = R.round_transforms >= tunable("expand_round_min", EXPAND_ROUND_MIN_DEFAULT) && R.digits_fit &&
                            (tree != 2 || tunable("expand_round_odd", 0) != 0);
    launch_ntt_inv(D.T, R.inv, s);
    if (one_launch) {
      launch_expand_round(D.T, R.es[0], R.es[1], s);
    } else {
      launch_ntt_fwd3(D.T, R.fd[0], R.fd[1], R.fd[2], s);
      launch_mac2(D.T, R.md[0], R.md[1], s);
    }
  }
}

void run_group_expansion(Workspace* const* Ws, const sp_pp* const* pps, int B, size_t g_rounds) {
  Workspace& W0 = *Ws[0];
  DeviceState& D = *W0.D;
  hipStream_t s = W0.stream;
  const int* L = D.lists.p;
  if (B < 1 || B > GROUP_MAX) throw ArgError("group size out of range");
  GroupOff g{};
  auto off = [](const void* q, const void* q0) { return (long long)((uintptr_t)q - (uintptr_t)q0); };
  for (int i = 0; i < B; i++) {
    Workspace& W = *Ws[i];
    if (W.P != W0.P || W.D != W0.D) throw ArgError("a group's queries must share params and device");
    g.v[i] = off(W.v.p, W0.v.p);
    g.raw[i] = off(W.exp_raw.p, W0.exp_raw.p);
    g.dig[i] = off(W.exp_dig.p, W0.exp_dig.p);
    g.ct1[i] = off(W.exp_ct1.p, W0.exp_ct1.p);
    g.pp[i] = off(pps[i]->all.p, pps[0]->all.p);
    if (pps[i]->has_right != pps[0]->has_right || pps[i]->off_left != pps[0]->off_left || pps[i]->off_right != pps[0]->off_right)
      throw ArgError("a group's public parameters must have one layout");
  }
  const long group_min = tunable("expand_group_round_min", EXPAND_GROUP_ROUND_MIN_DEFAULT);
  const long wave_min_digits = tunable("expand_wave_min_digits", EXPAND_WAVE_MIN_DIGITS_DEFAULT);
  bool wave_ok = wave_min_digits > 0;
  GroupOff gw = g;
  for (int i = 0; i < B; i++) {
    wave_ok = wave_ok && pps[i]->all_w.p != nullptr && pps[i]->all_w.n == pps[0]->all_w.n;
    if (wave_ok) gw.pp[i] = off(pps[i]->all_w.p, pps[0]->all_w.p);
  }
  for (size_t r = 0; r < g_rounds; r++) {
    const RoundPlan& rp = D.rounds[r];
    if (rp.n_all == 0 && rp.n_skip2 == 0) continue;
    const RoundLaunches R = round_launches(W0, *pps[0], rp, r, L, 0);
    launch_ntt_inv_group(D.T, R.inv, g, B, s);
    if (R.round_transforms * B >= group_min && R.digits_fit) {
      ExpandSideDesc coop[2] = {R.es[0], R.es[1]};
      for (int side = 1; side >= 0; side--)
        if (wave_ok && coop[side].cnt > 0 && coop[side].t >= wave_min_digits && coop[side].t <= 56) {
          ExpandWaveDesc w{};
          w.raw = coop[side].raw;
          w.pos = coop[side].pos;
          w.out_idx = coop[side].out_idx;
          w.A_w = pps[0]->all_w.p + (coop[side].A - pps[0]->all.p);
          w.const_w = pps[0]->all_w.p + pps[0]->all.n;
          w.v = coop[side].v;
          w.cnt = coop[side].cnt;
          w.t = coop[side].t;
          w.bits = coop[side].bits;
          launch_expand_wave(D.T, w, gw, B, s);
          coop[side].cnt = 0;
        }
      launch_expand_round_group(D.T, coop[0], coop[1], g, B, s);
    } else {
      launch_ntt_fwd3_group(D.T, R.fd[0], R.fd[1], R.fd[2], g, B, s);
      launch_mac2_group(D.T, R.md[0], R.md[1], g, B, s);
    }
  }
}

void run_regev_to_gsw(Workspace& W, const sp_pp& pp, const u32* v_src, const int* src_ct, const int* src_poly) {
  const Params& p = *W.P;
  DeviceState& D = *W.D;
  hipStream_t s = W.stream;
  const int* L = D.lists.p;
  const int nb = (int)(p.db_dim_2 * p.t_gsw);
  if (nb == 0) return;
  const int four_t = (int)(4 * p.t_gsw);
  launch_copy_polys(W.fold_mats.p, L + D.gsw_out_odd, four_t, v_src, src_poly, 1, 2, nb, s);
  InvDesc inv{};
  inv.src = v_src;
  inv.idx = src_ct;
  inv.polys_per_idx = 2;
  inv.idx_stride = 4 * POLY_LEN;
  inv.poly_stride = 2 * POLY_LEN;
  inv.crt_stride = POLY_LEN;
  inv.z_stride = 1;
  inv.dst = W.gsw_raw.p;
  inv.n_polys = nb * 2;
  launch_ntt_inv(D.T, inv, s);
  FwdDesc f{};
  f.src = W.gsw_raw.p;
  f.dst = W.gsw_dig.p;
  f.n_out = nb * 2 * (int)p.t_conv;
  f.rdim = 2;
  f.cols = 1;
  f.t = (int)p.t_conv;
  f.bits = (int)p.bits_per(p.t_conv);
  f.src_batch_stride = 2;
  f.src_row0 = 0;
  f.src_cols = 1;
  launch_ntt_fwd(D.T, f, s);
  MacDesc m{};
  m.A = pp.all.p + pp.off_conv * 2 * POLY_LEN;
  m.B = W.gsw_dig.p;
  m.out = W.fold_mats.p;
  m.out_idx = L + D.gsw_out_even;
  m.R = 2;
  m.K = 2 * (int)p.t_conv;
  m.batch_inner = nb;
  m.batch_outer = 1;
  m.B_inner_stride = 2 * p.t_conv;
  m.split_k = m.K;
  m.out_row_stride = four_t;
  launch_mac(D.T, m, s);
}

void run_folding_neg(Workspace& W) {
  const Params& p = *W.P;
  launch_folding_neg(W.D->T, W.fold_mats.p, W.D->gadget_gsw.p, (int)p.db_dim_2, (int)(2 * p.t_gsw), W.stream);
  run_mats_to_wave(W, p.db_dim_2);
}

void run_fold_operands(Workspace& W) {
  if (tunable("fold_neg_materialise", 0) != 0) {
    run_folding_neg(W);
    return;
  }
  run_mats_to_wave(W, W.P->db_dim_2, true);
}

void run_mats_to_wave(Workspace& W, size_t levels, bool c_only) {
  const Params& p = *W.P;
  W.mats_w_ready = false;
  if (tunable("fold_variant", FOLD_VARIANT_DEFAULT) != 5 || !fused_fold_supported(p) || levels == 0) return;
  const size_t words = levels * 2 * 4 * p.t_gsw * 2 * POLY_LEN;
  W.fold_mats_w.ensure(words);
  launch_mats_to_wave(W.fold_mats_w.p, W.fold_mats.p, words, W.stream, c_only ? (int)(2 * p.t_gsw) : 0);
  W.mats_w_ready = true;
}

void run_begin_direct(Workspace& W, const uint8_t* query) {
  const Params& p = *W.P;
  DeviceState& D = *W.D;
  hipStream_t s = W.stream;
  note_path(PATH_DIRECT_UPLOAD);
  const size_t dim0 = p.dim0(), nu2 = p.db_dim_2, two_t = 2 * p.t_gsw;
  const size_t n_reg = dim0 * POLY_LEN;
  const size_t gsw_polys = nu2 * 2 * two_t;
  const size_t n_rng = n_reg + nu2 * two_t * POLY_LEN;
  std::vector<u64> ks(n_rng);
  chacha20_keystream_u64(query, ks.data(), n_rng);
  for (auto& x : ks) x = p.modulus - (x % p.modulus);
  const uint8_t* wire = query + SEED_LENGTH;
  std::vector<u64> raw((dim0 + gsw_polys) * POLY_LEN);
  memcpy(raw.data(), ks.data(), n_reg * 8);
  const uint8_t* wire_gsw = wire + n_reg * 8;
  for (size_t d = 0; d < nu2; d++) {
    u64* m = raw.data() + (dim0 + d * 2 * two_t) * POLY_LEN;
    memcpy(m, ks.data() + n_reg + d * two_t * POLY_LEN, two_t * POLY_LEN * 8);
    memcpy(m + two_t * POLY_LEN, wire_gsw + d * two_t * POLY_LEN * 8, two_t * POLY_LEN * 8);
  }
  W.du_raw.ensure(raw.size());
  W.du_wire.ensure(n_reg);
  W.du_ntt.ensure((dim0 + gsw_polys) * 2 * POLY_LEN);
  W.qv.ensure(POLY_LEN * dim0 * 2);
  W.fold_mats.ensure(std::max<size_t>(nu2, 1) * 2 * 2 * two_t * 2 * POLY_LEN);
  HIP_CHECK(hipMemcpyAsync(W.du_raw.p, raw.data(), raw.size() * 8, hipMemcpyHostToDevice, s));
  HIP_CHECK(hipMemcpyAsync(W.du_wire.p, wire, n_reg * 8, hipMemcpyHostToDevice, s));
  FwdDesc f{W.du_raw.p, nullptr, W.du_ntt.p, (int)(dim0 + gsw_polys), 1, 1, 1, 64, 1, 0, 1};
  launch_ntt_fwd(D.T, f, s);
  launch_interleave_query(W.qv.p, W.du_ntt.p, W.du_wire.p, (int)dim0, s);
  const u32* gsw = W.du_ntt.p + dim0 * 2 * POLY_LEN;
  for (size_t d = 0; d < nu2; d++)
    for (size_t r = 0; r < 2; r++)
      HIP_CHECK(hipMemcpyAsync(W.fold_mats.p + ((d * 2 + r) * 2 * two_t + two_t) * 2 * POLY_LEN,
                               gsw + ((d * 2 + r) * two_t) * 2 * POLY_LEN, two_t * 2 * POLY_LEN * sizeof(u32),
                               hipMemcpyDeviceToDevice, s));
  run_fold_operands(W);
  HIP_CHECK(hipStreamSynchronize(s));
}

static void query_ct_host(Workspace& W, const uint8_t* query, size_t query_len, u64* host) {
  const Params& p = *W.P;
  if (query_len != p.query_bytes()) throw ArgError("query length " + std::to_string(query_len) + " != query_bytes " + std::to_string(p.query_bytes()));
  if (p.db_dim_2 == 0 && p.t_exp_left != p.t_exp_right) throw ArgError("nu_2 == 0 requires t_exp_left == t_exp_right (server.rs:573)");
  chacha20_keystream_u64(query, host, POLY_LEN);
  const FastMod modq(p.modulus);
  for (size_t i = 0; i < POLY_LEN; i++) host[i] = p.modulus - modq(host[i]);
  memcpy(host + POLY_LEN, query + SEED_LENGTH, POLY_LEN * sizeof(u64));
}

static void run_begin_query_ct(Workspace& W, const uint8_t* query, size_t query_len) {
  query_ct_host(W, query, query_len, W.h_query);
  W.ensure_expand();
  hipStream_t s = W.stream;
  join_right(W);
  W.right_pending = false;
  HIP_CHECK(hipMemcpyAsync(W.q_raw.p, W.h_query, 2 * POLY_LEN * sizeof(u64), hipMemcpyHostToDevice, s));
  FwdDesc f{W.q_raw.p, nullptr, W.v.p, 2, 1, 1, 1, 64, 1, 0, 1};
  launch_ntt_fwd(W.D->T, f, s);
}

static void run_begin_after_rounds(Workspace& W, const sp_pp& pp) {
  const Params& p = *W.P;
  DeviceState& D = *W.D;
  const int* L = D.lists.p;
  if (p.db_dim_2 > 0) {
    launch_reorient(W.qv.p, W.v.p, 0, 2, (int)p.dim0(), W.stream);
    run_regev_to_gsw(W, pp, W.v.p, L + D.gsw_src_ct, L + D.gsw_src_poly);
    run_fold_operands(W);
  } else {
    launch_reorient(W.qv.p, W.v.p, 0, 1, (int)p.dim0(), W.stream);
  }
}

static void run_group_after_rounds(Workspace* const* Ws, const sp_pp* const* pps, int B) {
  Workspace& W0 = *Ws[0];
  const Params& p = *W0.P;
  DeviceState& D = *W0.D;
  hipStream_t s = W0.stream;
  const int* L = D.lists.p;
  auto off = [](const void* q, const void* q0) { return (long long)((uintptr_t)q - (uintptr_t)q0); };
  const int nb = (int)(p.db_dim_2 * p.t_gsw);
  const int four_t = (int)(4 * p.t_gsw);
  const size_t mats_words = p.db_dim_2 * 2 * 4 * p.t_gsw * 2 * POLY_LEN;
  for (int i = 0; i < B; i++) Ws[i]->fold_mats_w.ensure(mats_words);
  GroupOff g_reo{}, g_copy{}, g_inv{}, g_fwd{}, g_mac{}, g_neg{}, g_wave{};
  for (int i = 0; i < B; i++) {
    Workspace& W = *Ws[i];
    const long long dv = off(W.v.p, W0.v.p), dm = off(W.fold_mats.p, W0.fold_mats.p);
    g_reo.v[i] = dv;   g_reo.raw[i] = off(W.qv.p, W0.qv.p);
    g_copy.v[i] = dv;  g_copy.raw[i] = dm;
    g_inv.v[i] = dv;   g_inv.raw[i] = off(W.gsw_raw.p, W0.gsw_raw.p);
    g_fwd.raw[i] = g_inv.raw[i];  g_fwd.dig[i] = off(W.gsw_dig.p, W0.gsw_dig.p);
    g_mac.pp[i] = off(pps[i]->all.p, pps[0]->all.p);  g_mac.dig[i] = g_fwd.dig[i];  g_mac.v[i] = dm;
    g_neg.v[i] = dm;
    g_wave.v[i] = dm;  g_wave.raw[i] = off(W.fold_mats_w.p, W0.fold_mats_w.p);
    if (pps[i]->off_conv != pps[0]->off_conv) throw ArgError("a group's public parameters must have one layout");
  }
  launch_reorient_group(W0.qv.p, W0.v.p, 0, 2, (int)p.dim0(), g_reo, B, s);
  if (nb > 0) {
    launch_copy_polys_group(W0.fold_mats.p, L + D.gsw_out_odd, four_t, W0.v.p, L + D.gsw_src_poly, 1, 2, nb, g_copy, B, s);
    InvDesc inv{};
    inv.src = W0.v.p;
    inv.idx = L + D.gsw_src_ct;
    inv.polys_per_idx = 2;
    inv.idx_stride = 4 * POLY_LEN;
    inv.poly_stride = 2 * POLY_LEN;
    inv.crt_stride = POLY_LEN;
    inv.z_stride = 1;
    inv.dst = W0.gsw_raw.p;
    inv.n_polys = nb * 2;
    launch_ntt_inv_group(D.T, inv, g_inv, B, s);
    FwdDesc f{};
    f.src = W0.gsw_raw.p;
    f.dst = W0.gsw_dig.p;
    f.n_out = nb * 2 * (int)p.t_conv;
    f.rdim = 2;
    f.cols = 1;
    f.t = (int)p.t_conv;
    f.bits = (int)p.bits_per(p.t_conv);
    f.src_batch_stride = 2;
    f.src_row0 = 0;
    f.src_cols = 1;
    FwdDesc none{};
    launch_ntt_fwd3_group(D.T, f, none, none, g_fwd, B, s);
    MacDesc m{};
    m.A = pps[0]->all.p + pps[0]->off_conv * 2 * POLY_LEN;
    m.B = W0.gsw_dig.p;
    m.out = W0.fold_mats.p;
    m.out_idx = L + D.gsw_out_even;
    m.R = 2;
    m.K = 2 * (int)p.t_conv;
    m.batch_inner = nb;
    m.batch_outer = 1;
    m.B_inner_stride = 2 * p.t_conv;
    m.split_k = m.K;
    m.out_row_stride = four_t;
    MacDesc none_m{};
    launch_mac2_group(D.T, m, none_m, g_mac, B, s);
  }
  const bool neg = tunable("fold_neg_materialise", 0) != 0;
  if (neg) launch_folding_neg_group(D.T, W0.fold_mats.p, D.gadget_gsw.p, (int)p.db_dim_2, (int)(2 * p.t_gsw), g_neg, B, s);
  launch_mats_to_wave_group(W0.fold_mats_w.p, W0.fold_mats.p, mats_words, neg ? 0 : (int)(2 * p.t_gsw), g_wave, B, s);
  for (int i = 0; i < B; i++) Ws[i]->mats_w_ready = true;
}

void run_begin_group(Workspace* const* Ws, const sp_pp* const* pps, const uint8_t* const* queries, const size_t* query_lens, int B) {
  Workspace& W0 = *Ws[0];
  const Params& p = *W0.P;
  if (!p.expand_queries) throw ArgError("run_begin_group: direct-upload queries have no expansion to share");
  if (!W0.h_group_query) {
    if (W0.host_pinned)
      HIP_CHECK(hipHostMalloc((void**)&W0.h_group_query, (size_t)GROUP_MAX * 2 * POLY_LEN * sizeof(u64), hipHostMallocDefault));
    else if (!(W0.h_group_query = (u64*)malloc((size_t)GROUP_MAX * 2 * POLY_LEN * sizeof(u64))))
      throw OomError("host staging allocation failed");
  }
  W0.group_q_raw.ensure((size_t)GROUP_MAX * 2 * POLY_LEN);
  GroupOff gq{};
  for (int i = 0; i < B; i++) {
    Workspace& W = *Ws[i];
    query_ct_host(W, queries[i], query_lens[i], W0.h_group_query + (size_t)i * 2 * POLY_LEN);
    W.ensure_expand();
    if (W.right_pending) {
      HIP_CHECK(hipStreamWaitEvent(W0.stream, W.ev_right, 0));
      W.right_pending = false;
    }
    gq.raw[i] = (long long)((size_t)i * 2 * POLY_LEN * sizeof(u64));
    gq.dig[i] = (long long)((uintptr_t)W.v.p - (uintptr_t)W0.v.p);
  }
  HIP_CHECK(hipMemcpyAsync(W0.group_q_raw.p, W0.h_group_query, (size_t)B * 2 * POLY_LEN * sizeof(u64), hipMemcpyHostToDevice, W0.stream));
  {
    FwdDesc f{W0.group_q_raw.p, nullptr, W0.v.p, 2, 1, 1, 1, 64, 1, 0, 1};
    FwdDesc none{};
    launch_ntt_fwd3_group(W0.D->T, f, none, none, gq, B, W0.stream);
  }
  note_path(PATH_EXPAND_GROUP);
  run_group_expansion(Ws, pps, B, p.g());
  if (tunable("expand_group_tail", 1) != 0 && fused_fold_supported(p) && tunable("fold_variant", FOLD_VARIANT_DEFAULT) == 5 && p.db_dim_2 > 0)
    run_group_after_rounds(Ws, pps, B);
  else
    for (int i = 0; i < B; i++) {
      Workspace& W = *Ws[i];
      hipStream_t own = W.stream;
      W.stream = W0.stream;
      try {
        run_begin_after_rounds(W, *pps[i]);
      } catch (...) {
        W.stream = own;
        throw;
      }
      W.stream = own;
    }
  HIP_CHECK(hipEventRecord(W0.ev_round0, W0.stream));
  for (int i = 1; i < B; i++) HIP_CHECK(hipStreamWaitEvent(Ws[i]->stream, W0.ev_round0, 0));
}

void run_begin(Workspace& W, const sp_pp& pp, const uint8_t* query, size_t query_len, int j0, int nj,
               const DeviceState::PrunedPlan* plan) {
  const Params& p = *W.P;
  DeviceState& D = *W.D;
  if (query_len != p.query_bytes()) throw ArgError("query length " + std::to_string(query_len) + " != query_bytes " + std::to_string(p.query_bytes()));
  if (!p.expand_queries) {
    run_begin_direct(W, query);
    return;
  }
  run_begin_query_ct(W, query, query_len);
  hipStream_t s = W.stream;
  const size_t g = p.g();
  const bool prune = p.db_dim_2 > 0 && nj > 0 && (j0 != 0 || nj != (int)p.dim0());
  if (prune || (plan && p.db_dim_2 > 0)) note_path(PATH_EXPAND_PRUNED);
  const DeviceState::PrunedPlan* pl = plan && p.db_dim_2 > 0 ? plan : (prune ? &D.pruned_plan(p, j0, nj) : nullptr);
  const int* L = D.lists.p;
  const long split_mode = tunable("expand_split", -1);
  if (p.db_dim_2 > 0 && g >= 2 && (split_mode > 0 || (split_mode < 0 && W.long_sweep_follows))) {
    note_path(PATH_EXPAND_SPLIT);
    run_coefficient_expansion(W, pp, 1, pl, 0, 0);
    HIP_CHECK(hipEventRecord(W.ev_round0, s));
    HIP_CHECK(hipStreamWaitEvent(W.stream2, W.ev_round0, 0));
    on_stream(W, W.stream2, [&] {
      run_coefficient_expansion(W, pp, g, pl, 2, 1);
      run_regev_to_gsw(W, pp, W.v.p, L + D.gsw_src_ct, L + D.gsw_src_poly);
      run_fold_operands(W);
    });
    HIP_CHECK(hipEventRecord(W.ev_right, W.stream2));
    W.right_pending = true;
    run_coefficient_expansion(W, pp, g, pl, 1, 1);
    launch_reorient(W.qv.p, W.v.p, 0, 2, (int)p.dim0(), s);
    return;
  }
  run_coefficient_expansion(W, pp, g, pl);
  run_begin_after_rounds(W, pp);
}

void join_right(Workspace& W) {
  if (W.right_pending) HIP_CHECK(hipStreamWaitEvent(W.stream, W.ev_right, 0));
}

void run_sweep(Workspace& W, const sp_db& db) {
  if (db.planar_resident) throw ArgError("the single-query sweep kernels do not read a planar-resident database (sp_db_create_planar)");
  const Params& p = *W.P;
  W.ensure_sweep();
  SweepDesc d{db.words.p, W.qv.p, W.sweep_out.p, (int)p.planes(), db.np_local, (int)p.dim0(), db.j0, db.nj, db.packed, W.out_G};
  d.nt_store = (int)tunable("sweep_nt_store", 1);
  launch_sweep(W.D->T, d, W.stream);
}

void run_sweep_sparse(Workspace& W, const sp_db& db, const int* col_ptr, const int* col_rows, const int* col_slots) {
  const Params& p = *W.P;
  W.ensure_sweep();
  launch_sweep_sparse(W.D->T, col_ptr, col_rows, col_slots, db.polys.p, (int)p.planes(), W.v.p, 0,
                      p.db_dim_2 > 0 ? 2 : 1, W.sweep_out.p, (int)p.num_per(), W.stream);
}

void run_sweep_sparse_group(Workspace* const* Ws, int B, const sp_db& db, const int* col_ptr, const int* col_rows, const int* col_slots,
                            hipStream_t s) {
  const Params& p = *Ws[0]->P;
  SparseGroup g{};
  for (int b = 0; b < B; b++) {
    Ws[b]->ensure_sweep();
    g.v[b] = Ws[b]->v.p;
    g.out[b] = Ws[b]->sweep_out.p;
  }
  launch_sweep_sparse_batch(Ws[0]->D->T, col_ptr, col_rows, col_slots, db.polys.p, (int)p.planes(), g, B, 0, p.db_dim_2 > 0 ? 2 : 1,
                            (int)p.num_per(), s);
}

void run_sweep_sparse_scatter(Workspace& W, const sp_db& db, const int* col_ptr, const int* col_rows, const int* col_slots, int G,
                              int plane0, int n_planes, bool per_plane) {
  const Params& p = *W.P;
  W.ensure_sweep();
  launch_sweep_sparse_scatter(W.D->T, col_ptr, col_rows, col_slots, db.polys.p, (int)p.planes(), plane0, n_planes, W.v.p, 0,
                              p.db_dim_2 > 0 ? 2 : 1, W.sweep_out.p, (int)p.num_per(), G, per_plane, W.stream);
}
void run_sweep_sparse_scatter_group(Workspace* const* Ws, int B, const sp_db& db, const int* col_ptr, const int* col_rows,
                                    const int* col_slots, int G, hipStream_t s) {
  const Params& p = *Ws[0]->P;
  SparseGroup g{};
  for (int b = 0; b < B; b++) {
    Ws[b]->ensure_sweep();
    g.v[b] = Ws[b]->v.p;
    g.out[b] = Ws[b]->sweep_out.p;
  }
  launch_sweep_sparse_scatter_batch(Ws[0]->D->T, col_ptr, col_rows, col_slots, db.polys.p, (int)p.planes(), g, B, 0,
                                    p.db_dim_2 > 0 ? 2 : 1, (int)p.num_per(), G, s);
}

static FoldOpts query_fold_opts(const Workspace& W, bool below_q) {
  return FoldOpts{std::min(W.fused_min_pairs, tunable("fused_min_pairs_cap", 1L << 62)), true, below_q};
}

static void fold_planes(Workspace& W, size_t pg0, int np, bool premod) {
  const Params& p = *W.P;
  DeviceState& D = *W.D;
  hipStream_t s = W.stream;
  if (p.num_per() % 4 == 0 && !tunable("from_sweep1", 0)) {
    launch_from_sweep4(D.T, W.sweep_out.p + pg0 * 4 * POLY_LEN * p.num_per(), (int)p.num_per(), np, premod ? 1 : 0,
                       W.foldX.p, s);
  } else {
    InvDesc inv{};
    inv.src = W.sweep_out.p + pg0 * 4 * POLY_LEN * p.num_per();
    inv.sweep_np = (int)p.num_per();
    inv.dst = W.foldX.p;
    inv.n_polys = np * (int)p.num_per() * 2;
    inv.premod = premod ? 1 : 0;
    launch_ntt_inv(D.T, inv, s);
  }
  u64* res = run_fold(W, query_fold_opts(W, true), W.foldX.p, W.foldY.p, np, (int)p.num_per(), -1);
  HIP_CHECK(hipMemcpyAsync(W.final_cts.p + pg0 * 2 * POLY_LEN, res, (size_t)np * 2 * POLY_LEN * sizeof(u64), hipMemcpyDeviceToDevice, s));
}

static int tail_defer_levels(const Params& p, long stop) {
  if (stop <= 0 || !fused_fold_supported(p) || p.planes() < 2) return 0;
  int lv = 0;
  size_t cur = p.num_per();
  while (cur > (size_t)stop && cur / 2 >= 1 && (cur & 1) == 0) { cur >>= 1; lv++; }
  return cur == (size_t)stop && lv > 0 && stop >= 2 ? lv : 0;
}
static void fold_plane_head(Workspace& W, size_t pl, int levels) {
  const Params& p = *W.P;
  launch_from_sweep4(W.D->T, W.sweep_out.p + pl * 4 * POLY_LEN * p.num_per(), (int)p.num_per(), 1, 0, W.foldX.p, W.stream);
  u64* res = run_fold(W, query_fold_opts(W, true), W.foldX.p, W.foldY.p, 1, (int)p.num_per(), -1, 0, levels);
  const size_t cts = p.num_per() >> levels;
  HIP_CHECK(hipMemcpyAsync(W.fold_tail.p + pl * cts * 2 * POLY_LEN, res, cts * 2 * POLY_LEN * sizeof(u64), hipMemcpyDeviceToDevice, W.stream));
}
static void fold_tails(Workspace& W, int levels) {
  const Params& p = *W.P;
  const size_t cts = p.num_per() >> levels;
  u64* other = W.fold_tail.p + p.planes() * cts * 2 * POLY_LEN;
  u64* res = run_fold(W, query_fold_opts(W, true), W.fold_tail.p, other, (int)p.planes(), (int)p.num_per(), -1, levels, -1);
  HIP_CHECK(hipMemcpyAsync(W.final_cts.p, res, p.planes() * 2 * POLY_LEN * sizeof(u64), hipMemcpyDeviceToDevice, W.stream));
}

bool sweep_is_pipelined(const Params& p, const sp_db& db) {
  const bool enabled = tunable("pipeline", 1) != 0;
  return enabled && db.packed && db.num_shards == 1 && db.col_G == 1 && p.planes() > 1 && p.num_per() >= 1024;
}

void launch_plane_sweep(Workspace& W, const sp_db& db, size_t pl) {
  if (db.planar_resident) throw ArgError("the single-query sweep kernels do not read a planar-resident database (sp_db_create_planar)");
  const Params& p = *W.P;
  const size_t np_ = (size_t)db.np_local;
  const size_t plane_db_words = db_bytes(1, db.np_local, db.nj, db.packed) / 8;
  SweepDesc d{db.words.p + pl * plane_db_words, W.qv.p, W.sweep_out.p + pl * 4 * POLY_LEN * np_, 1, db.np_local,
              (int)p.dim0(), db.j0, db.nj, db.packed, W.out_G};
  d.nt_store = (int)tunable("sweep_nt_store", 1);
  const int wgs = (int)tunable("pipe_wgs", 4);
  if (db.packed && wgs > 0)
    launch_sweep_persist(W.D->T, d, wgs, W.stream);
  else
    launch_sweep(W.D->T, d, W.stream);
}

void run_sweep_pipelined(Workspace& W, const sp_db& db) {
  const Params& p = *W.P;
  W.ensure_sweep();
  W.ensure_finish();
  const size_t planes = p.planes();
  HIP_CHECK(hipEventRecord(W.ev_sw[0], W.stream));
  const int defer_levels = tail_defer_levels(p, tunable("pipe_tail_defer", 256));
  if (defer_levels > 0) {
    W.fold_tail.ensure(2 * planes * (p.num_per() >> defer_levels) * 2 * POLY_LEN);
    note_path(PATH_FOLD_TAIL_BATCHED);
  }
  for (size_t pl = 0; pl < planes; pl++) {
    launch_plane_sweep(W, db, pl);
    HIP_CHECK(hipEventRecord(W.ev_plane[pl], W.stream));
    HIP_CHECK(hipStreamWaitEvent(W.stream2, W.ev_plane[pl], 0));
    if (defer_levels > 0) {
      on_stream(W, W.stream2, [&] {
        fold_plane_head(W, pl, defer_levels);
        if (pl + 1 == planes) fold_tails(W, defer_levels);
      });
      continue;
    }
    on_stream(W, W.stream2, [&] { fold_planes(W, pl, 1, false); });
  }
  HIP_CHECK(hipEventRecord(W.ev_sw[1], W.stream));
  HIP_CHECK(hipEventRecord(W.ev_fold, W.stream2));
  W.have_sweep_span = true;
  W.pipelined = true;
  note_path(PATH_PIPELINED);
}

bool fused_fold_supported(const Params& p) { return 4 * p.t_gsw <= 128 && p.bits_per(p.t_gsw) <= 28; }

u64* run_fold(Workspace& W, const FoldOpts& o, u64* X, u64* Y, int np, int num_cts, int top, int d_begin, int d_end) {
  const Params& p = *W.P;
  DeviceState& D = *W.D;
  hipStream_t s = W.stream;
  const int two_t = (int)(2 * p.t_gsw);
  join_right(W);
  int further = 0;
  while (((int)1 << further) < num_cts) further++;
  const int top_idx = top < 0 ? further - 1 : top;
  if (d_end < 0) d_end = further;
  int cur = num_cts >> d_begin;
  for (int d = d_begin; d < d_end; d++) {
    const int half = cur / 2;
    if (W.zero_shortcuts && !fused_fold_supported(p))
      throw ArgError("sparse buckets need gadget parameters the fused fold supports (3 <= t_gsw <= 32)");
    if (W.zero_shortcuts || ((long)np * half >= o.fused_min_pairs && fused_fold_supported(p))) {
      FoldDesc fd{};
      fd.zero_shortcuts = W.zero_shortcuts ? 1 : 0;
      fd.mats_w = W.mats_w_ready ? W.fold_mats_w.p + (size_t)(top_idx - d) * 2 * 2 * two_t * 2 * POLY_LEN : nullptr;
      fd.X = X;
      fd.Y = Y;
      fd.mats = W.fold_mats.p + (size_t)(top_idx - d) * 2 * 2 * two_t * 2 * POLY_LEN;
      fd.cur = cur;
      fd.half = half;
      fd.planes = np;
      fd.t = (int)p.t_gsw;
      fd.bits = (int)p.bits_per(p.t_gsw);
      fd.t_live = o.inputs_below_q && tunable("fold_skip_dead_digits", 1)
                      ? (int)std::min<size_t>(p.t_gsw, (p.modulus_log2 + fd.bits - 1) / fd.bits) : fd.t;
      launch_fold_fused(D.T, fd, s);
      std::swap(X, Y);
      cur = half;
      continue;
    }
    if (o.delta_tail) {
      FwdDesc f{};
      f.src = X;
      f.dst = W.fold_dig.p;
      f.n_out = np * half * two_t;
      f.rdim = 2;
      f.cols = 1;
      f.t = (int)p.t_gsw;
      f.bits = (int)p.bits_per(p.t_gsw);
      f.src_batch_stride = 2;
      f.src_row0 = 0;
      f.src_cols = 1;
      f.delta_off = (long)half * 2;
      f.delta_inner = half;
      f.delta_outer_stride = cur;
      launch_ntt_fwd(D.T, f, s);
      MacDesc m{};
      m.A = W.fold_mats.p + ((size_t)(top_idx - d) * 2 * 2 * two_t + two_t) * 2 * POLY_LEN;
      m.A_row_stride = 2 * two_t;
      m.B = W.fold_dig.p;
      m.out = W.fold_ntt.p;
      m.R = 2;
      m.K = two_t;
      m.batch_inner = np * half;
      m.batch_outer = 1;
      m.B_inner_stride = two_t;
      m.split_k = two_t;
      m.out_batch_stride = 2;
      m.out_row_stride = 1;
      launch_mac(D.T, m, s);
      InvDesc inv{};
      inv.src = W.fold_ntt.p;
      inv.poly_stride = 2 * POLY_LEN;
      inv.crt_stride = POLY_LEN;
      inv.z_stride = 1;
      inv.dst = Y;
      inv.n_polys = np * half * 2;
      inv.addend = X;
      inv.add_inner2 = half * 2;
      inv.add_outer_stride = cur * 2;
      launch_ntt_inv(D.T, inv, s);
      note_path(PATH_FOLD_TAIL);
      std::swap(X, Y);
      cur = half;
      continue;
    }
    FwdDesc f{};
    f.src = X;
    f.dst = W.fold_dig.p;
    f.n_out = np * cur * two_t;
    f.rdim = 2;
    f.cols = 1;
    f.t = (int)p.t_gsw;
    f.bits = (int)p.bits_per(p.t_gsw);
    f.src_batch_stride = 2;
    f.src_row0 = 0;
    f.src_cols = 1;
    launch_ntt_fwd(D.T, f, s);
    MacDesc m{};
    m.A = W.fold_mats.p + (size_t)(top_idx - d) * 2 * 2 * two_t * 2 * POLY_LEN;
    m.B = W.fold_dig.p;
    m.out = W.fold_ntt.p;
    m.R = 2;
    m.K = 2 * two_t;
    m.batch_inner = half;
    m.batch_outer = np;
    m.B_inner_stride = two_t;
    m.B_outer_stride = (long)cur * two_t;
    m.split_k = two_t;
    m.split_off = (long)half * two_t;
    m.out_batch_stride = 2;
    m.out_row_stride = 1;
    launch_mac(D.T, m, s);
    InvDesc inv{};
    inv.src = W.fold_ntt.p;
    inv.poly_stride = 2 * POLY_LEN;
    inv.crt_stride = POLY_LEN;
    inv.z_stride = 1;
    inv.dst = Y;
    inv.n_polys = np * half * 2;
    launch_ntt_inv(D.T, inv, s);
    note_path(PATH_FOLD_TAIL_LITERAL);
    std::swap(X, Y);
    cur = half;
  }
  return X;
}

static void run_pack_v1(Workspace& W, const sp_pp& pp) {
  const Params& p = *W.P;
  DeviceState& D = *W.D;
  hipStream_t s = W.stream;
  const int* L = D.lists.p;
  const int tc = (int)p.t_conv;
  note_path(PATH_PACK_V1);
  const int nb = (int)p.planes();
  const int ne = (int)p.instances * 2;
  const size_t PW = 2 * POLY_LEN;
  W.pack_v1_P.ensure((size_t)nb * 3 * PW);
  W.pack_v1_P2.ensure((size_t)ne * 3 * PW);
  W.pack_v1_raw.ensure((size_t)ne * POLY_LEN);
  const u32* w_key = pp.all.p + (pp.off_packing + 0 * 3 * tc) * PW;
  const u32* w_shift = pp.all.p + (pp.off_packing + 1 * 3 * tc) * PW;
  FwdDesc f{};
  f.src = W.final_cts.p;
  f.src_idx = L + D.pack_src_ct;
  f.dst = W.pack_dig.p;
  f.n_out = nb * tc;
  f.rdim = 1; f.cols = 1; f.t = tc; f.bits = (int)p.bits_per(tc);
  f.src_batch_stride = 2; f.src_row0 = 0; f.src_cols = 1;
  launch_ntt_fwd(D.T, f, s);
  MacDesc m{};
  m.A = w_key; m.B = W.pack_dig.p; m.out = W.pack_v1_P.p;
  m.R = 3; m.K = tc; m.batch_inner = nb; m.batch_outer = 1; m.B_inner_stride = tc; m.split_k = tc;
  m.out_batch_stride = 3; m.out_row_stride = 1;
  launch_mac(D.T, m, s);
  FwdDesc f2 = f;
  f2.dst = W.pack_ct2.p; f2.n_out = nb; f2.t = 1; f2.bits = 64; f2.src_row0 = 1;
  launch_ntt_fwd(D.T, f2, s);
  launch_add_poly_into(D.T, W.pack_v1_P.p, L + D.v1_row1, W.pack_ct2.p, nb, s);
  InvDesc inv{};
  inv.src = W.pack_v1_P.p; inv.idx = L + D.v1_shift_src; inv.polys_per_idx = 1;
  inv.idx_stride = (long)PW; inv.poly_stride = (long)PW; inv.crt_stride = POLY_LEN; inv.z_stride = 1;
  inv.dst = W.pack_v1_raw.p; inv.n_polys = ne;
  launch_ntt_inv(D.T, inv, s);
  FwdDesc f3{};
  f3.src = W.pack_v1_raw.p; f3.dst = W.pack_dig.p; f3.n_out = ne * tc;
  f3.rdim = 1; f3.cols = 1; f3.t = tc; f3.bits = (int)p.bits_per(tc);
  f3.src_batch_stride = 1; f3.src_row0 = 0; f3.src_cols = 1;
  launch_ntt_fwd(D.T, f3, s);
  MacDesc m2 = m;
  m2.A = w_shift; m2.out = W.pack_v1_P2.p; m2.batch_inner = ne;
  launch_mac(D.T, m2, s);
  launch_add_polys_idx(D.T, W.pack_v1_P2.p, L + D.v1_rot_dst, W.pack_v1_P2.p, L + D.v1_rot_a, W.pack_v1_P.p, L + D.v1_rot_b, 2 * ne, s);
  launch_add_polys_idx(D.T, W.pack_res.p, L + D.v1_sum_dst, W.pack_v1_P.p, L + D.v1_sum_a, W.pack_v1_P2.p, L + D.v1_sum_b, 3 * ne, s);
  InvDesc inv2{};
  inv2.src = W.pack_res.p; inv2.poly_stride = (long)PW; inv2.crt_stride = POLY_LEN; inv2.z_stride = 1;
  inv2.dst = W.pack_raw.p; inv2.n_polys = (int)(p.instances * 3 * 2);
  launch_ntt_inv(D.T, inv2, s);
}

void run_pack(Workspace& W, const sp_pp& pp) {
  const Params& p = *W.P;
  if (p.version == 1) {
    run_pack_v1(W, pp);
    return;
  }
  DeviceState& D = *W.D;
  hipStream_t s = W.stream;
  const int* L = D.lists.p;
  const int n = (int)p.n, tc = (int)p.t_conv;
  const int nb = (int)p.planes();
  FwdDesc f{};
  f.src = W.final_cts.p;
  f.src_idx = L + D.pack_src_ct;
  f.dst = W.pack_dig.p;
  f.n_out = nb * tc;
  f.rdim = 1;
  f.cols = 1;
  f.t = tc;
  f.bits = (int)p.bits_per(tc);
  f.src_batch_stride = 2;
  f.src_row0 = 0;
  f.src_cols = 1;
  launch_ntt_fwd(D.T, f, s);
  MacDesc m{};
  m.A = pp.pack_cat.p;
  m.B = W.pack_dig.p;
  m.out = W.pack_res.p;
  m.out_idx = L + D.pack_out;
  m.R = n + 1;
  m.K = n * tc;
  m.batch_inner = (int)p.instances * n;
  m.batch_outer = 1;
  m.B_inner_stride = (long)n * tc;
  m.split_k = m.K;
  m.out_row_stride = n;
  launch_mac(D.T, m, s);
  FwdDesc f2 = f;
  f2.dst = W.pack_ct2.p;
  f2.n_out = nb;
  f2.t = 1;
  f2.bits = 64;
  f2.src_row0 = 1;
  launch_ntt_fwd(D.T, f2, s);
  launch_add_poly_into(D.T, W.pack_res.p, L + D.pack_row, W.pack_ct2.p, nb, s);
  InvDesc inv{};
  inv.src = W.pack_res.p;
  inv.poly_stride = 2 * POLY_LEN;
  inv.crt_stride = POLY_LEN;
  inv.z_stride = 1;
  inv.dst = W.pack_raw.p;
  inv.n_polys = (int)(p.instances * (p.n + 1) * p.n);
  launch_ntt_inv(D.T, inv, s);
}

void run_fold_all(Workspace& W, bool premod) {
  const Params& p = *W.P;
  const size_t pg = W.plane_group();
  for (size_t pg0 = 0; pg0 < p.planes(); pg0 += pg) fold_planes(W, pg0, (int)std::min(pg, p.planes() - pg0), premod);
}

static inline u64 rescale_coeff(u64 a, u64 inp_mod, u64 out_mod) {
  typedef __int128 i128;
  const int64_t im = (int64_t)inp_mod;
  int64_t v = (int64_t)(a % inp_mod);
  if (v >= im / 2) v -= im;
  const int64_t sign = v >= 0 ? 1 : -1;
  i128 num = (i128)v * (i128)out_mod + (i128)(sign * (im / 2));
  i128 res = num / (i128)inp_mod;
  const i128 om = (i128)out_mod;
  res = (res + (i128)((inp_mod / out_mod) * out_mod) + 2 * om) % om;
  return (u64)((res + om) % om);
}

size_t encode_response(const Params& p, const u64* packed, uint8_t* out) {
  const u64 q1 = 4 * p.pt_modulus;
  size_t q1_bits = 0;
  while (((u64)1 << q1_bits) < q1) q1_bits++;
  const u64 q2 = p.q2();
  const size_t q2_bits = p.q2_bits;
  const size_t total = p.response_bytes();
  memset(out, 0, total);
  u64* w = reinterpret_cast<u64*>(out);
  (void)w;
  std::vector<u64> words(total / 8, 0);
  size_t bit = 0;
  auto put = [&](u64 val, size_t nbits) {
    val &= (nbits >= 64) ? ~0ULL : (((u64)1 << nbits) - 1);
    size_t wi = bit >> 6, off = bit & 63;
    words[wi] |= val << off;
    if (off + nbits > 64) words[wi + 1] |= val >> (64 - off);
    bit += nbits;
  };
  const size_t mat = (p.n + 1) * p.n * POLY_LEN;
  for (size_t inst = 0; inst < p.instances; inst++) {
    const u64* m = packed + inst * mat;
    for (size_t i = 0; i < p.n * POLY_LEN; i++) put(rescale_coeff(m[i], p.modulus, q2), q2_bits);
    const u64* rest = m + p.n * POLY_LEN;
    for (size_t i = 0; i < p.n * p.n * POLY_LEN; i++) put(rescale_coeff(rest[i], p.modulus, q1), q1_bits);
  }
  memcpy(out, words.data(), total);
  return total;
}

static void fold_local_planes(Workspace& W, const u32* chunk, int G, size_t pg0, int np) {
  const Params& p = *W.P;
  DeviceState& D = *W.D;
  hipStream_t s = W.stream;
  const int npl = (int)p.num_per() / G;
  if (npl % 4 == 0) {
    launch_from_sweep4(D.T, chunk, npl, np, 1, W.foldX.p, s);
  } else {
    InvDesc inv{};
    inv.src = chunk;
    inv.sweep_np = npl;
    inv.dst = W.foldX.p;
    inv.n_polys = np * npl * 2;
    inv.premod = 1;
    launch_ntt_inv(D.T, inv, s);
  }
  u64* res = run_fold(W, query_fold_opts(W, true), W.foldX.p, W.foldY.p, np, npl, (int)p.db_dim_2 - 1);
  HIP_CHECK(hipMemcpyAsync(W.final_cts.p + pg0 * 2 * POLY_LEN, res, (size_t)np * 2 * POLY_LEN * sizeof(u64), hipMemcpyDeviceToDevice, s));
}

void run_fold_local(Workspace& W, const u32* reduced_chunk, int G) {
  const Params& p = *W.P;
  W.ensure_finish();
  const int npl = (int)p.num_per() / G;
  const size_t pg = W.plane_group();
  for (size_t pg0 = 0; pg0 < p.planes(); pg0 += pg)
    fold_local_planes(W, reduced_chunk + pg0 * 4 * POLY_LEN * npl, G, pg0, (int)std::min(pg, p.planes() - pg0));
}

void run_fold_local_plane(Workspace& W, const u32* reduced_plane_chunk, int G, int plane) {
  W.ensure_finish();
  std::swap(W.stream, W.stream2);
  try {
    fold_local_planes(W, reduced_plane_chunk, G, (size_t)plane, 1);
  } catch (...) {
    std::swap(W.stream, W.stream2);
    throw;
  }
  std::swap(W.stream, W.stream2);
}

void run_fold_local_join(Workspace& W) {
  HIP_CHECK(hipEventRecord(W.ev_fold, W.stream2));
  HIP_CHECK(hipStreamWaitEvent(W.stream, W.ev_fold, 0));
}

void run_finish_gathered(Workspace& W, const sp_pp& pp, const u64* gathered, int G) {
  const Params& p = *W.P;
  hipStream_t s = W.stream;
  W.ensure_finish();
  const size_t ctw = 2 * POLY_LEN;
  const int planes = (int)p.planes();
  W.foldX.ensure((size_t)planes * G * ctw);
  W.foldY.ensure((size_t)planes * std::max(G / 2, 1) * ctw);
  HIP_CHECK(hipMemcpy2DAsync(W.foldX.p, (size_t)G * ctw * 8, gathered, ctw * 8, ctw * 8, (size_t)planes, hipMemcpyDeviceToDevice, s));
  for (int g = 1; g < G; g++)
    HIP_CHECK(hipMemcpy2DAsync(W.foldX.p + (size_t)g * ctw, (size_t)G * ctw * 8, gathered + (size_t)g * planes * ctw, ctw * 8,
                               ctw * 8, (size_t)planes, hipMemcpyDeviceToDevice, s));
  int lg = 0;
  while ((1 << lg) < G) lg++;
  u64* res = run_fold(W, query_fold_opts(W, false), W.foldX.p, W.foldY.p, planes, G, lg - 1);
  HIP_CHECK(hipMemcpyAsync(W.final_cts.p, res, (size_t)planes * ctw * sizeof(u64), hipMemcpyDeviceToDevice, s));
  HIP_CHECK(hipEventRecord(W.ev[3], s));
  run_pack(W, pp);
  run_encode_device(W);
  HIP_CHECK(hipEventRecord(W.ev[4], s));
}

void run_encode_device(Workspace& W) {
  const Params& p = *W.P;
  hipStream_t s = W.stream;
  HIP_CHECK(hipMemsetAsync(W.enc_out.p, 0, W.enc_out.bytes(), s));
  EncodeDesc e{};
  e.packed = W.pack_raw.p;
  e.out = reinterpret_cast<unsigned long long*>(W.enc_out.p);
  e.instances = (int)p.instances;
  e.n = (int)p.n;
  e.Q = p.modulus;
  e.q1 = 4 * p.pt_modulus;
  e.q2 = p.q2();
  int q1_bits = 0;
  while (((u64)1 << q1_bits) < e.q1) q1_bits++;
  e.q1_bits = q1_bits;
  e.q2_bits = (int)p.q2_bits;
  launch_encode(e, s);
  HIP_CHECK(hipMemcpyAsync(W.h_response, W.enc_out.p, p.response_bytes(), hipMemcpyDeviceToHost, s));
}

void run_finish(Workspace& W, const sp_pp& pp, bool premod) {
  const Params& p = *W.P;
  W.ensure_finish();
  if (W.pipelined) {
    HIP_CHECK(hipStreamWaitEvent(W.stream, W.ev_fold, 0));
    W.pipelined = false;
  } else {
    run_fold_all(W, premod);
  }
  HIP_CHECK(hipEventRecord(W.ev[3], W.stream));
  run_pack(W, pp);
  run_encode_device(W);
  HIP_CHECK(hipEventRecord(W.ev[4], W.stream));
  (void)p;
}

}
```

sdk_amd/csrc/server.hpp:

```cpp
#pragma once
#include <cstdio>
#include <cstdlib>
#include <hip/hip_runtime.h>

#include <memory>
#include <mutex>
#include <stdexcept>
#include <string>
#include <unordered_map>
#include <vector>

#include "kernels.hpp"
#include "params.hpp"

namespace spiral {

struct HipError : std::runtime_error {
  explicit HipError(const std::string& s) : std::runtime_error(s) {}
};
struct ArgError : std::runtime_error {
  explicit ArgError(const std::string& s) : std::runtime_error(s) {}
};
struct OomError : std::runtime_error {
  explicit OomError(const std::string& s) : std::runtime_error(s) {}
};

void hip_check(hipError_t e, const char* what, const char* file, int line);
#define HIP_CHECK(x) ::spiral::hip_check((x), #x, __FILE__, __LINE__)
u64 paths_taken(bool reset);
void set_tunable(const char* name, long v);
void tunables_new_call();
void devbuf_fresh(void* p, size_t bytes);
void* devbuf_alloc(size_t bytes, size_t* guard, long* serial);
void devbuf_free(void* p, size_t bytes, size_t guard, long serial);
bool devbuf_guards_on();
void devbuf_cache_sync();

template <typename T>
struct DevBuf {
  T* p = nullptr;
  size_t n = 0;
  size_t guard = 0;
  long serial = -1;
  DevBuf() {}
  explicit DevBuf(size_t count) { alloc(count); }
  DevBuf(const DevBuf&) = delete;
  DevBuf& operator=(const DevBuf&) = delete;
  DevBuf(DevBuf&& o) noexcept : p(o.p), n(o.n), guard(o.guard), serial(o.serial) { o.p = nullptr; o.n = 0; o.guard = 0; }
  DevBuf& operator=(DevBuf&& o) noexcept {
    if (this != &o) { release(); p = o.p; n = o.n; guard = o.guard; serial = o.serial; o.p = nullptr; o.n = 0; o.guard = 0; }
    return *this;
  }
  ~DevBuf() { release(); }
  void alloc(size_t count) {
    release();
    if (count == 0) return;
    void* q = devbuf_alloc(count * sizeof(T), &guard, &serial);
    p = (T*)q;
    n = count;
  }
  void alloc_streaming(size_t count, bool want_contiguous) {
    release();
    if (count == 0) return;
    if (want_contiguous && !devbuf_guards_on()) {
      void* q = nullptr;
      const hipError_t e = hipExtMallocWithFlags(&q, count * sizeof(T), hipDeviceMallocContiguous);
      if (getenv("SPIRAL_ALLOC_DEBUG")) fprintf(stderr, "[spiral] contiguous allocation of %zu bytes: %s -> [%p, %p)\n", count * sizeof(T), hipGetErrorName(e), q, (char*)q + count * sizeof(T));
      if (e == hipSuccess && q) {
        p = (T*)q;
        n = count;
        devbuf_cache_sync();
        (void)hipDeviceSynchronize();
        return;
      }
      (void)hipGetLastError();
    }
    alloc(count);
  }
  void ensure(size_t count) { if (count > n) alloc(count); }
  void release() { if (p) { devbuf_free(p, n * sizeof(T), guard, serial); p = nullptr; n = 0; guard = 0; serial = -1; } }
  size_t bytes() const { return n * sizeof(T); }
};

void upload_words(void* dst, const void* host, size_t bytes);
void h2d_sync(void* dst, const void* host, size_t bytes);

void chacha20_keystream_u64(const uint8_t seed[32], u64* out, size_t count);

struct RoundPlan {
  int num_in = 0, t_auto = 0;
  int n_all = 0, n_left = 0, n_right = 0;
  size_t all_ct = 0;
  size_t all_row1 = 0;
  size_t left_pos = 0;
  size_t left_out = 0;
  size_t right_pos = 0, right_out = 0;
  size_t left_ct = 0, right_ct = 0;
  size_t skip2 = 0;
  int n_skip2 = 0;
};

struct DeviceState {
  int device = -1;
  DevTables T;
  DevBuf<u32> tw;
  DevBuf<u32> neg1;
  DevBuf<u32> gadget_gsw;
  DevBuf<int> lists;
  std::vector<RoundPlan> rounds;
  std::vector<RoundPlan> rounds_even, rounds_odd;
  size_t max_all = 0, max_left = 0, max_right = 0;
  struct PrunedPlan {
    int j0 = 0, nj = 0;
    std::vector<RoundPlan> rounds;
    std::vector<RoundPlan> rounds_even, rounds_odd;
    DevBuf<int> lists;
  };
  std::vector<std::unique_ptr<PrunedPlan>> pruned;
  std::mutex pruned_mu;
  const PrunedPlan& pruned_plan(const Params& P, int j0, int nj);
  size_t gsw_src_ct = 0;
  size_t gsw_src_poly = 0;
  size_t gsw_out_even = 0;
  size_t gsw_out_odd = 0;
  size_t pack_src_ct = 0;
  size_t pack_out = 0;
  size_t pack_row = 0;
  size_t v1_row1 = 0;
  size_t v1_shift_src = 0;
  size_t v1_rot_dst = 0, v1_rot_a = 0, v1_rot_b = 0;
  size_t v1_sum_dst = 0, v1_sum_a = 0, v1_sum_b = 0;
  struct PpExpand {
    std::mutex mu;
    DevBuf<u64> table, raw;
    hipStream_t stream = nullptr;
    ~PpExpand() {
      if (stream) {
        (void)hipStreamSynchronize(stream);
        (void)hipStreamDestroy(stream);
      }
    }
  } pp_expand;
};

struct Workspace;

}

struct sp_params {
  spiral::Params p;
  std::mutex mu;
  std::vector<std::unique_ptr<spiral::DeviceState>> dev;
  std::vector<std::unique_ptr<spiral::Workspace>> ws_pool;
  spiral::DeviceState& device_state();
  std::unique_ptr<spiral::Workspace> acquire_ws();
  void release_ws(std::unique_ptr<spiral::Workspace> ws);
  ~sp_params();
};

struct sp_pp {
  const sp_params* params = nullptr;
  int device = -1;
  spiral::DevBuf<spiral::u32> all;
  size_t n_polys = 0;
  size_t off_packing = 0, off_left = 0, off_right = 0, off_conv = 0;
  bool has_right = false;
  spiral::DevBuf<spiral::u32> pack_cat;
  spiral::DevBuf<spiral::u32> all_w;
};

struct sp_ppc {
  const sp_params* params = nullptr;
  int device = -1;
  spiral::DevBuf<uint8_t> image;
};

struct sp_db {
  const sp_params* params = nullptr;
  int device = -1;
  int shard = 0, num_shards = 1;
  int j0 = 0, nj = 0;
  int packed = 0;
  int col_g = 0, col_G = 1;
  int np_local = 0;
  spiral::ColMap colmap() const { return spiral::ColMap{col_g, col_G, np_local * col_G}; }
  spiral::DevBuf<spiral::u64> words;
  std::shared_ptr<spiral::DevBuf<spiral::u64>> planar;
  int planar_state = 0;
  std::shared_ptr<const spiral::DevBuf<spiral::u64>> ensure_planar(hipStream_t s);
  void drop_planar() {
    if (planar_state != -1) planar_state = 0;
    planar.reset();
  }
  bool planar_resident = false;
  std::mutex mu;
  struct WriteScope {
    sp_db& d;
    std::lock_guard<std::mutex> lk;
    explicit WriteScope(sp_db& db) : d(db), lk(db.mu) {}
    ~WriteScope() { d.drop_planar(); }
  };
  bool sparse = false;
  std::unordered_map<size_t, size_t> slot_of;
  spiral::DevBuf<spiral::u64> polys;
  size_t slots_cap = 0;
  bool index_dirty = true;
  bool rows_dirty = true;
  struct SparseIndex {
    spiral::DevBuf<int> col_ptr, col_rows, col_slots;
    std::shared_ptr<spiral::DeviceState::PrunedPlan> plan;
  };
  std::shared_ptr<const SparseIndex> sparse_index;
  spiral::DevBuf<uint8_t> upload;
  std::shared_ptr<const SparseIndex> ensure_sparse_index();
  struct ReadBack {
    std::mutex mu;
    spiral::DevBuf<uint8_t> buf;
    hipStream_t stream = nullptr;
    ~ReadBack() {
      if (stream) {
        (void)hipStreamSynchronize(stream);
        (void)hipStreamDestroy(stream);
      }
    }
  };
  mutable ReadBack readback;
};
```

Baseline: 89.86 queries/s.

## Fuse pack add into MAC, write fold output in place, shared-memory encode

The separate add_poly_into kernel is removed: the row-1 ciphertext is NTT'd in the same launch as the digits and added inside the MAC through a generalized extra/extra_per path. run_fold can write its last level straight into the final buffer, which drops trailing device-to-device copies. Encode now packs each block's bits in shared memory, so the global memset and global atomics go away. In pipelined mode, pack and encode run on stream2 instead of waiting on a fold event. The change also adds begin-phase host timing instrumentation and splits coefficient expansion into two calls. Together these mainly trim small tail-path launches and copies, while the per-query cost is dominated by the sweep over the 56 GiB database.

```diff
diff --git a/sdk_amd/csrc/bodies.hpp b/sdk_amd/csrc/bodies.hpp
--- a/sdk_amd/csrc/bodies.hpp
+++ b/sdk_amd/csrc/bodies.hpp
@@ -171,7 +171,8 @@
     const u32* A = d.A + (size_t)r * (d.A_row_stride ? d.A_row_stride : d.K) * PW + e;
     const long op = (ob + (long)r * d.out_row_stride) * 2 * N + e;
     u64 acc = d.addend ? (u64)d.addend[op] : 0ULL;
-    if (d.extra && r == d.extra_row) acc += (u64)d.extra[(size_t)(d.extra_idx ? d.extra_idx[b] : b) * PW + e];
+    const int er = r - d.extra_row, ep = d.extra_per ? d.extra_per : 1;
+    if (d.extra && er >= 0 && er < ep) acc += (u64)d.extra[((size_t)(d.extra_idx ? d.extra_idx[b] : b) * ep + er) * PW + e];
     for (int seg = 0; seg < 2; seg++) {
       const int k_lo = seg == 0 ? 0 : d.split_k, k_hi = seg == 0 ? min(d.split_k, d.K) : d.K;
       const u32* Bs = seg == 0 ? B : B + (size_t)(d.split_off - d.split_k) * PW;
@@ -211,13 +212,6 @@
     }
     d.out[op] = (u32)acc;
   }
-}
-
-__device__ __forceinline__ void add_poly_into_body(const DevTables& T, u32* dst, const int* idx, const u32* src, int b, int ychunk) {
-  const int e = ychunk * 256 + threadIdx.x;
-  const int c = e >> POLY_LEN_LOG2;
-  const long dp = (long)idx[b] * 2 * N + e;
-  dst[dp] = add_mod(dst[dp], src[(size_t)b * 2 * N + e], T.c.mod[c].q);
 }
 
 __device__ __forceinline__ void copy_polys_body(const CopyPolysDesc& d, int bx, int ychunk) {
@@ -300,32 +294,28 @@
   return (r + out_mod) % out_mod;
 }
 
-__device__ __forceinline__ void encode_body(const EncodeDesc& d, int blk) {
+__device__ __forceinline__ void encode_body(const EncodeDesc& d, int blk, unsigned long long* words) {
   const int per_inst_first = d.n * N, per_inst_rest = d.n * d.n * N;
   const int per_inst = per_inst_first + per_inst_rest;
-  const long i = (long)blk * 256 + threadIdx.x;
-  if (i >= (long)d.instances * per_inst) return;
-  const int inst = (int)(i / per_inst), k = (int)(i % per_inst);
+  const int tid = threadIdx.x;
+  const long i0 = (long)blk * 256;
+  const int inst = (int)(i0 / per_inst), k0 = (int)(i0 % per_inst);
   const u64* m = d.packed + (size_t)inst * (d.n + 1) * d.n * N;
-  const size_t inst_bits = (size_t)per_inst_first * d.q2_bits + (size_t)per_inst_rest * d.q1_bits;
-  u64 val;
-  size_t bit;
-  int nb;
-  if (k < per_inst_first) {
-    val = rescale_dev(m[k], d.Q, d.q2);
-    nb = d.q2_bits;
-    bit = (size_t)inst * inst_bits + (size_t)k * d.q2_bits;
-  } else {
-    const int kk = k - per_inst_first;
-    val = rescale_dev(m[per_inst_first + kk], d.Q, d.q1);
-    nb = d.q1_bits;
-    bit = (size_t)inst * inst_bits + (size_t)per_inst_first * d.q2_bits + (size_t)kk * d.q1_bits;
-  }
+  const size_t first_bits = (size_t)per_inst_first * d.q2_bits;
+  const size_t inst_bits = first_bits + (size_t)per_inst_rest * d.q1_bits;
+  const bool first = k0 < per_inst_first;
+  const int nb = first ? d.q2_bits : d.q1_bits;
+  const size_t run_bit = (size_t)inst * inst_bits + (first ? (size_t)k0 * d.q2_bits : first_bits + (size_t)(k0 - per_inst_first) * d.q1_bits);
+  const int n_words = 4 * nb;
+  if (tid < n_words) words[tid] = 0;
+  __syncthreads();
+  u64 val = rescale_dev(m[k0 + tid], d.Q, first ? d.q2 : d.q1);
   val &= nb >= 64 ? ~0ULL : ((1ULL << nb) - 1ULL);
-  const size_t w = bit >> 6;
-  const int off = (int)(bit & 63);
-  atomicOr(d.out + w, (unsigned long long)(val << off));
-  if (off + nb > 64) atomicOr(d.out + w + 1, (unsigned long long)(val >> (64 - off)));
-}
-
-}
+  const int off = tid * nb, w = off >> 6, o = off & 63;
+  atomicOr(words + w, (unsigned long long)(val << o));
+  if (o + nb > 64) atomicOr(words + w + 1, (unsigned long long)(val >> (64 - o)));
+  __syncthreads();
+  if (tid < n_words) d.out[(run_bit >> 6) + tid] = words[tid];
+}
+
+}
diff --git a/sdk_amd/csrc/elementwise.hip b/sdk_amd/csrc/elementwise.hip
--- a/sdk_amd/csrc/elementwise.hip
+++ b/sdk_amd/csrc/elementwise.hip
@@ -48,15 +48,6 @@
   launched(0, "k_mac2");
 }
 
-__global__ __launch_bounds__(256) void k_add_poly_into(DevTables T, u32* dst, const int* idx, const u32* src) {
-  add_poly_into_body(T, dst, idx, src, blockIdx.x, blockIdx.y);
-}
-void launch_add_poly_into(const DevTables& T, u32* dst, const int* idx, const u32* src, int batch, hipStream_t s) {
-  if (batch <= 0) return;
-  hipLaunchKernelGGL(k_add_poly_into, dim3(batch, 2 * N / 256), dim3(256), 0, s, T, dst, idx, src);
-  launched(0, "k_add_poly_into");
-}
-
 __global__ __launch_bounds__(256) void k_scalar_mul(DevTables T, u32* base, long dst_off, long src_off,
                                                     const u32* scalar) {
   const int e = blockIdx.y * 256 + threadIdx.x;
@@ -251,7 +242,10 @@
   launched(0, "k_u32_to_u64");
 }
 
-__global__ __launch_bounds__(256) void k_encode(EncodeDesc d) { encode_body(d, blockIdx.x); }
+__global__ __launch_bounds__(256) void k_encode(EncodeDesc d) {
+  __shared__ unsigned long long words[256];
+  encode_body(d, blockIdx.x, words);
+}
 void launch_encode(const EncodeDesc& d, hipStream_t s) {
   const long total = (long)d.instances * ((long)d.n * N + (long)d.n * d.n * N);
   hipLaunchKernelGGL(k_encode, dim3((unsigned)((total + 255) / 256)), dim3(256), 0, s, d);
diff --git a/sdk_amd/csrc/kernels.hpp b/sdk_amd/csrc/kernels.hpp
--- a/sdk_amd/csrc/kernels.hpp
+++ b/sdk_amd/csrc/kernels.hpp
@@ -127,6 +127,7 @@
   const u32* extra;
   const int* extra_idx;
   int extra_row;
+  int extra_per;
 };
 void launch_mac(const DevTables& T, const MacDesc& d, hipStream_t s);
 void launch_mac2(const DevTables& T, const MacDesc& d0, const MacDesc& d1, hipStream_t s);
@@ -185,7 +186,6 @@
 constexpr long FOLD_VARIANT_DEFAULT = 5;
 void launch_fold_fused(const DevTables& T, const FoldDesc& d, hipStream_t s);
 
-void launch_add_poly_into(const DevTables& T, u32* dst, const int* idx, const u32* src, int batch, hipStream_t s);
 void launch_scalar_mul(const DevTables& T, u32* base, long dst_off, long src_off, const u32* scalar, int n_polys,
                        hipStream_t s);
 void launch_add_polys_idx(const DevTables& T, u32* dst, const int* di, const u32* a, const int* ai, const u32* b,
@@ -238,12 +238,6 @@
   const u32* src;
   size_t n_words;
   int half_polys;
-};
-struct AddPolyIntoDesc {
-  u32* dst;
-  const int* idx;
-  const u32* src;
-  int batch;
 };
 struct CopyWordsDesc {
   u32* dst;
diff --git a/sdk_amd/csrc/pipeline.hpp b/sdk_amd/csrc/pipeline.hpp
--- a/sdk_amd/csrc/pipeline.hpp
+++ b/sdk_amd/csrc/pipeline.hpp
@@ -1,4 +1,5 @@
 #pragma once
+#include <chrono>
 #include <vector>
 
 #include "server.hpp"
@@ -16,6 +17,9 @@
   hipEvent_t ev_round0 = nullptr, ev_right = nullptr;
   bool right_pending = false;
   bool long_sweep_follows = false;
+  bool begin_trace = false;
+  std::chrono::steady_clock::time_point begin_t0;
+  double begin_us[4] = {0, 0, 0, 0};
   hipEvent_t ev_sw[2] = {nullptr, nullptr};
   bool have_sweep_span = false;
   bool pipelined = false;
@@ -91,7 +95,8 @@
   bool delta_tail;
   bool inputs_below_q;
 };
-u64* run_fold(Workspace& W, const FoldOpts& o, u64* X, u64* Y, int np, int num_cts, int top, int d_begin = 0, int d_end = -1);
+u64* run_fold(Workspace& W, const FoldOpts& o, u64* X, u64* Y, int np, int num_cts, int top, int d_begin = 0, int d_end = -1,
+              u64* last_dst = nullptr);
 void run_fold_local(Workspace& W, const u32* reduced_chunk, int G);
 void run_fold_local_plane(Workspace& W, const u32* reduced_plane_chunk, int G, int plane);
 void run_fold_local_join(Workspace& W);
diff --git a/sdk_amd/csrc/server.cpp b/sdk_amd/csrc/server.cpp
--- a/sdk_amd/csrc/server.cpp
+++ b/sdk_amd/csrc/server.cpp
@@ -449,24 +449,19 @@
     D->gsw_out_odd = put(out_odd);
   }
   {
-    std::vector<int> src_ct, out, row;
+    std::vector<int> src_ct, out;
     const int n = (int)P.n;
     for (int inst = 0; inst < (int)P.instances; inst++)
       for (int c = 0; c < n; c++) {
         out.push_back(inst * (n + 1) * n + c);
-        for (int r = 0; r < n; r++) {
-          src_ct.push_back(inst * n * n + r * n + c);
-          row.push_back(inst * (n + 1) * n + (1 + r) * n + c);
-        }
+        for (int r = 0; r < n; r++) src_ct.push_back(inst * n * n + r * n + c);
       }
     D->pack_src_ct = put(src_ct);
     D->pack_out = put(out);
-    D->pack_row = put(row);
   }
   if (P.version == 1 && P.n == 2) {
-    std::vector<int> row1, ssrc, rd, ra, rb, sd, sa, sb;
+    std::vector<int> ssrc, rd, ra, rb, sd, sa, sb;
     const int ne = (int)P.instances * 2;
-    for (int b = 0; b < ne * 2; b++) row1.push_back(b * 3 + 1);
     for (int e = 0; e < ne; e++) {
       const int inst = e / 2, c = e % 2, b0 = e * 2, b1 = e * 2 + 1;
       ssrc.push_back(b1 * 3);
@@ -478,7 +473,6 @@
         sb.push_back(e * 3 + rr);
       }
     }
-    D->v1_row1 = put(row1);
     D->v1_shift_src = put(ssrc);
     D->v1_rot_dst = put(rd); D->v1_rot_a = put(ra); D->v1_rot_b = put(rb);
     D->v1_sum_dst = put(sd); D->v1_sum_a = put(sa); D->v1_sum_b = put(sb);
@@ -654,6 +648,14 @@
 }
 
 void join_right(Workspace& W);
+
+static void begin_trace_sweep(Workspace& W) {
+  if (!W.begin_trace) return;
+  W.begin_trace = false;
+  const double t = std::chrono::duration<double, std::micro>(std::chrono::steady_clock::now() - W.begin_t0).count();
+  fprintf(stderr, "begin_host_times us: round0 %.1f even_first %.1f even_last %.1f reorient %.1f sweep0 %.1f\n", W.begin_us[0],
+          W.begin_us[1], W.begin_us[2], W.begin_us[3], t);
+}
 
 struct RoundLaunches {
   InvDesc inv;
@@ -1104,6 +1106,8 @@
   const Params& p = *W.P;
   DeviceState& D = *W.D;
   if (query_len != p.query_bytes()) throw ArgError("query length " + std::to_string(query_len) + " != query_bytes " + std::to_string(p.query_bytes()));
+  W.begin_trace = false;
+  W.begin_t0 = std::chrono::steady_clock::now();
   if (!p.expand_queries) {
     run_begin_direct(W, query);
     return;
@@ -1118,7 +1122,12 @@
   const long split_mode = tunable("expand_split", -1);
   if (p.db_dim_2 > 0 && g >= 2 && (split_mode > 0 || (split_mode < 0 && W.long_sweep_follows))) {
     note_path(PATH_EXPAND_SPLIT);
+    W.begin_trace = tunable("begin_host_times", 0) != 0;
+    auto mark = [&](int k) {
+      if (W.begin_trace) W.begin_us[k] = std::chrono::duration<double, std::micro>(std::chrono::steady_clock::now() - W.begin_t0).count();
+    };
     run_coefficient_expansion(W, pp, 1, pl, 0, 0);
+    mark(0);
     HIP_CHECK(hipEventRecord(W.ev_round0, s));
     HIP_CHECK(hipStreamWaitEvent(W.stream2, W.ev_round0, 0));
     on_stream(W, W.stream2, [&] {
@@ -1128,8 +1137,12 @@
     });
     HIP_CHECK(hipEventRecord(W.ev_right, W.stream2));
     W.right_pending = true;
-    run_coefficient_expansion(W, pp, g, pl, 1, 1);
+    run_coefficient_expansion(W, pp, 2, pl, 1, 1);
+    mark(1);
+    run_coefficient_expansion(W, pp, g, pl, 1, 2);
+    mark(2);
     launch_reorient(W.qv.p, W.v.p, 0, 2, (int)p.dim0(), s);
+    mark(3);
     return;
   }
   run_coefficient_expansion(W, pp, g, pl);
@@ -1147,6 +1160,7 @@
   SweepDesc d{db.words.p, W.qv.p, W.sweep_out.p, (int)p.planes(), db.np_local, (int)p.dim0(), db.j0, db.nj, db.packed, W.out_G};
   d.nt_store = (int)tunable("sweep_nt_store", 1);
   launch_sweep(W.D->T, d, W.stream);
+  begin_trace_sweep(W);
 }
 
 void run_sweep_sparse(Workspace& W, const sp_db& db, const int* col_ptr, const int* col_rows, const int* col_slots) {
@@ -1209,8 +1223,9 @@
     inv.premod = premod ? 1 : 0;
     launch_ntt_inv(D.T, inv, s);
   }
-  u64* res = run_fold(W, query_fold_opts(W, true), W.foldX.p, W.foldY.p, np, (int)p.num_per(), -1);
-  HIP_CHECK(hipMemcpyAsync(W.final_cts.p + pg0 * 2 * POLY_LEN, res, (size_t)np * 2 * POLY_LEN * sizeof(u64), hipMemcpyDeviceToDevice, s));
+  u64* const dst = W.final_cts.p + pg0 * 2 * POLY_LEN;
+  u64* res = run_fold(W, query_fold_opts(W, true), W.foldX.p, W.foldY.p, np, (int)p.num_per(), -1, 0, -1, dst);
+  if (res != dst) HIP_CHECK(hipMemcpyAsync(dst, res, (size_t)np * 2 * POLY_LEN * sizeof(u64), hipMemcpyDeviceToDevice, s));
 }
 
 static int tail_defer_levels(const Params& p, long stop) {
@@ -1223,16 +1238,18 @@
 static void fold_plane_head(Workspace& W, size_t pl, int levels) {
   const Params& p = *W.P;
   launch_from_sweep4(W.D->T, W.sweep_out.p + pl * 4 * POLY_LEN * p.num_per(), (int)p.num_per(), 1, 0, W.foldX.p, W.stream);
-  u64* res = run_fold(W, query_fold_opts(W, true), W.foldX.p, W.foldY.p, 1, (int)p.num_per(), -1, 0, levels);
   const size_t cts = p.num_per() >> levels;
-  HIP_CHECK(hipMemcpyAsync(W.fold_tail.p + pl * cts * 2 * POLY_LEN, res, cts * 2 * POLY_LEN * sizeof(u64), hipMemcpyDeviceToDevice, W.stream));
+  u64* const park = W.fold_tail.p + pl * cts * 2 * POLY_LEN;
+  u64* res = run_fold(W, query_fold_opts(W, true), W.foldX.p, W.foldY.p, 1, (int)p.num_per(), -1, 0, levels, park);
+  if (res != park) HIP_CHECK(hipMemcpyAsync(park, res, cts * 2 * POLY_LEN * sizeof(u64), hipMemcpyDeviceToDevice, W.stream));
 }
 static void fold_tails(Workspace& W, int levels) {
   const Params& p = *W.P;
   const size_t cts = p.num_per() >> levels;
   u64* other = W.fold_tail.p + p.planes() * cts * 2 * POLY_LEN;
-  u64* res = run_fold(W, query_fold_opts(W, true), W.fold_tail.p, other, (int)p.planes(), (int)p.num_per(), -1, levels, -1);
-  HIP_CHECK(hipMemcpyAsync(W.final_cts.p, res, p.planes() * 2 * POLY_LEN * sizeof(u64), hipMemcpyDeviceToDevice, W.stream));
+  u64* res = run_fold(W, query_fold_opts(W, true), W.fold_tail.p, other, (int)p.planes(), (int)p.num_per(), -1, levels, -1, W.final_cts.p);
+  if (res != W.final_cts.p)
+    HIP_CHECK(hipMemcpyAsync(W.final_cts.p, res, p.planes() * 2 * POLY_LEN * sizeof(u64), hipMemcpyDeviceToDevice, W.stream));
 }
 
 bool sweep_is_pipelined(const Params& p, const sp_db& db) {
@@ -1253,6 +1270,7 @@
     launch_sweep_persist(W.D->T, d, wgs, W.stream);
   else
     launch_sweep(W.D->T, d, W.stream);
+  begin_trace_sweep(W);
 }
 
 void run_sweep_pipelined(Workspace& W, const sp_db& db) {
@@ -1280,7 +1298,6 @@
     on_stream(W, W.stream2, [&] { fold_planes(W, pl, 1, false); });
   }
   HIP_CHECK(hipEventRecord(W.ev_sw[1], W.stream));
-  HIP_CHECK(hipEventRecord(W.ev_fold, W.stream2));
   W.have_sweep_span = true;
   W.pipelined = true;
   note_path(PATH_PIPELINED);
@@ -1288,7 +1305,7 @@
 
 bool fused_fold_supported(const Params& p) { return 4 * p.t_gsw <= 128 && p.bits_per(p.t_gsw) <= 28; }
 
-u64* run_fold(Workspace& W, const FoldOpts& o, u64* X, u64* Y, int np, int num_cts, int top, int d_begin, int d_end) {
+u64* run_fold(Workspace& W, const FoldOpts& o, u64* X, u64* Y, int np, int num_cts, int top, int d_begin, int d_end, u64* last_dst) {
   const Params& p = *W.P;
   DeviceState& D = *W.D;
   hipStream_t s = W.stream;
@@ -1301,6 +1318,7 @@
   int cur = num_cts >> d_begin;
   for (int d = d_begin; d < d_end; d++) {
     const int half = cur / 2;
+    u64* const out = last_dst && d + 1 == d_end ? last_dst : Y;
     if (W.zero_shortcuts && !fused_fold_supported(p))
       throw ArgError("sparse buckets need gadget parameters the fused fold supports (3 <= t_gsw <= 32)");
     if (W.zero_shortcuts || ((long)np * half >= o.fused_min_pairs && fused_fold_supported(p))) {
@@ -1308,7 +1326,7 @@
       fd.zero_shortcuts = W.zero_shortcuts ? 1 : 0;
       fd.mats_w = W.mats_w_ready ? W.fold_mats_w.p + (size_t)(top_idx - d) * 2 * 2 * two_t * 2 * POLY_LEN : nullptr;
       fd.X = X;
-      fd.Y = Y;
+      fd.Y = out;
       fd.mats = W.fold_mats.p + (size_t)(top_idx - d) * 2 * 2 * two_t * 2 * POLY_LEN;
       fd.cur = cur;
       fd.half = half;
@@ -1318,7 +1336,8 @@
       fd.t_live = o.inputs_below_q && tunable("fold_skip_dead_digits", 1)
                       ? (int)std::min<size_t>(p.t_gsw, (p.modulus_log2 + fd.bits - 1) / fd.bits) : fd.t;
       launch_fold_fused(D.T, fd, s);
-      std::swap(X, Y);
+      Y = X;
+      X = out;
       cur = half;
       continue;
     }
@@ -1357,14 +1376,15 @@
       inv.poly_stride = 2 * POLY_LEN;
       inv.crt_stride = POLY_LEN;
       inv.z_stride = 1;
-      inv.dst = Y;
+      inv.dst = out;
       inv.n_polys = np * half * 2;
       inv.addend = X;
       inv.add_inner2 = half * 2;
       inv.add_outer_stride = cur * 2;
       launch_ntt_inv(D.T, inv, s);
       note_path(PATH_FOLD_TAIL);
-      std::swap(X, Y);
+      Y = X;
+      X = out;
       cur = half;
       continue;
     }
@@ -1400,11 +1420,12 @@
     inv.poly_stride = 2 * POLY_LEN;
     inv.crt_stride = POLY_LEN;
     inv.z_stride = 1;
-    inv.dst = Y;
+    inv.dst = out;
     inv.n_polys = np * half * 2;
     launch_ntt_inv(D.T, inv, s);
     note_path(PATH_FOLD_TAIL_LITERAL);
-    std::swap(X, Y);
+    Y = X;
+    X = out;
     cur = half;
   }
   return X;
@@ -1432,16 +1453,15 @@
   f.n_out = nb * tc;
   f.rdim = 1; f.cols = 1; f.t = tc; f.bits = (int)p.bits_per(tc);
   f.src_batch_stride = 2; f.src_row0 = 0; f.src_cols = 1;
-  launch_ntt_fwd(D.T, f, s);
+  FwdDesc f2 = f;
+  f2.dst = W.pack_ct2.p; f2.n_out = nb; f2.t = 1; f2.bits = 64; f2.src_row0 = 1;
+  launch_ntt_fwd3(D.T, f, f2, FwdDesc{}, s);
   MacDesc m{};
   m.A = w_key; m.B = W.pack_dig.p; m.out = W.pack_v1_P.p;
   m.R = 3; m.K = tc; m.batch_inner = nb; m.batch_outer = 1; m.B_inner_stride = tc; m.split_k = tc;
   m.out_batch_stride = 3; m.out_row_stride = 1;
+  m.extra = W.pack_ct2.p; m.extra_row = 1;
   launch_mac(D.T, m, s);
-  FwdDesc f2 = f;
-  f2.dst = W.pack_ct2.p; f2.n_out = nb; f2.t = 1; f2.bits = 64; f2.src_row0 = 1;
-  launch_ntt_fwd(D.T, f2, s);
-  launch_add_poly_into(D.T, W.pack_v1_P.p, L + D.v1_row1, W.pack_ct2.p, nb, s);
   InvDesc inv{};
   inv.src = W.pack_v1_P.p; inv.idx = L + D.v1_shift_src; inv.polys_per_idx = 1;
   inv.idx_stride = (long)PW; inv.poly_stride = (long)PW; inv.crt_stride = POLY_LEN; inv.z_stride = 1;
@@ -1453,7 +1473,7 @@
   f3.src_batch_stride = 1; f3.src_row0 = 0; f3.src_cols = 1;
   launch_ntt_fwd(D.T, f3, s);
   MacDesc m2 = m;
-  m2.A = w_shift; m2.out = W.pack_v1_P2.p; m2.batch_inner = ne;
+  m2.A = w_shift; m2.out = W.pack_v1_P2.p; m2.batch_inner = ne; m2.extra = nullptr;
   launch_mac(D.T, m2, s);
   launch_add_polys_idx(D.T, W.pack_v1_P2.p, L + D.v1_rot_dst, W.pack_v1_P2.p, L + D.v1_rot_a, W.pack_v1_P.p, L + D.v1_rot_b, 2 * ne, s);
   launch_add_polys_idx(D.T, W.pack_res.p, L + D.v1_sum_dst, W.pack_v1_P.p, L + D.v1_sum_a, W.pack_v1_P2.p, L + D.v1_sum_b, 3 * ne, s);
@@ -1486,7 +1506,13 @@
   f.src_batch_stride = 2;
   f.src_row0 = 0;
   f.src_cols = 1;
-  launch_ntt_fwd(D.T, f, s);
+  FwdDesc f2 = f;
+  f2.dst = W.pack_ct2.p;
+  f2.n_out = nb;
+  f2.t = 1;
+  f2.bits = 64;
+  f2.src_row0 = 1;
+  launch_ntt_fwd3(D.T, f, f2, FwdDesc{}, s);
   MacDesc m{};
   m.A = pp.pack_cat.p;
   m.B = W.pack_dig.p;
@@ -1499,15 +1525,10 @@
   m.B_inner_stride = (long)n * tc;
   m.split_k = m.K;
   m.out_row_stride = n;
+  m.extra = W.pack_ct2.p;
+  m.extra_row = 1;
+  m.extra_per = n;
   launch_mac(D.T, m, s);
-  FwdDesc f2 = f;
-  f2.dst = W.pack_ct2.p;
-  f2.n_out = nb;
-  f2.t = 1;
-  f2.bits = 64;
-  f2.src_row0 = 1;
-  launch_ntt_fwd(D.T, f2, s);
-  launch_add_poly_into(D.T, W.pack_res.p, L + D.pack_row, W.pack_ct2.p, nb, s);
   InvDesc inv{};
   inv.src = W.pack_res.p;
   inv.poly_stride = 2 * POLY_LEN;
@@ -1583,8 +1604,9 @@
     inv.premod = 1;
     launch_ntt_inv(D.T, inv, s);
   }
-  u64* res = run_fold(W, query_fold_opts(W, true), W.foldX.p, W.foldY.p, np, npl, (int)p.db_dim_2 - 1);
-  HIP_CHECK(hipMemcpyAsync(W.final_cts.p + pg0 * 2 * POLY_LEN, res, (size_t)np * 2 * POLY_LEN * sizeof(u64), hipMemcpyDeviceToDevice, s));
+  u64* const dst = W.final_cts.p + pg0 * 2 * POLY_LEN;
+  u64* res = run_fold(W, query_fold_opts(W, true), W.foldX.p, W.foldY.p, np, npl, (int)p.db_dim_2 - 1, 0, -1, dst);
+  if (res != dst) HIP_CHECK(hipMemcpyAsync(dst, res, (size_t)np * 2 * POLY_LEN * sizeof(u64), hipMemcpyDeviceToDevice, s));
 }
 
 void run_fold_local(Workspace& W, const u32* reduced_chunk, int G) {
@@ -1627,8 +1649,8 @@
                                ctw * 8, (size_t)planes, hipMemcpyDeviceToDevice, s));
   int lg = 0;
   while ((1 << lg) < G) lg++;
-  u64* res = run_fold(W, query_fold_opts(W, false), W.foldX.p, W.foldY.p, planes, G, lg - 1);
-  HIP_CHECK(hipMemcpyAsync(W.final_cts.p, res, (size_t)planes * ctw * sizeof(u64), hipMemcpyDeviceToDevice, s));
+  u64* res = run_fold(W, query_fold_opts(W, false), W.foldX.p, W.foldY.p, planes, G, lg - 1, 0, -1, W.final_cts.p);
+  if (res != W.final_cts.p) HIP_CHECK(hipMemcpyAsync(W.final_cts.p, res, (size_t)planes * ctw * sizeof(u64), hipMemcpyDeviceToDevice, s));
   HIP_CHECK(hipEventRecord(W.ev[3], s));
   run_pack(W, pp);
   run_encode_device(W);
@@ -1638,7 +1660,6 @@
 void run_encode_device(Workspace& W) {
   const Params& p = *W.P;
   hipStream_t s = W.stream;
-  HIP_CHECK(hipMemsetAsync(W.enc_out.p, 0, W.enc_out.bytes(), s));
   EncodeDesc e{};
   e.packed = W.pack_raw.p;
   e.out = reinterpret_cast<unsigned long long*>(W.enc_out.p);
@@ -1659,11 +1680,17 @@
   const Params& p = *W.P;
   W.ensure_finish();
   if (W.pipelined) {
-    HIP_CHECK(hipStreamWaitEvent(W.stream, W.ev_fold, 0));
     W.pipelined = false;
-  } else {
-    run_fold_all(W, premod);
-  }
+    HIP_CHECK(hipEventRecord(W.ev[3], W.stream2));
+    on_stream(W, W.stream2, [&] {
+      run_pack(W, pp);
+      run_encode_device(W);
+    });
+    HIP_CHECK(hipEventRecord(W.ev[4], W.stream2));
+    HIP_CHECK(hipStreamWaitEvent(W.stream, W.ev[4], 0));
+    return;
+  }
+  run_fold_all(W, premod);
   HIP_CHECK(hipEventRecord(W.ev[3], W.stream));
   run_pack(W, pp);
   run_encode_device(W);
diff --git a/sdk_amd/csrc/server.hpp b/sdk_amd/csrc/server.hpp
--- a/sdk_amd/csrc/server.hpp
+++ b/sdk_amd/csrc/server.hpp
@@ -125,8 +125,6 @@
   size_t gsw_out_odd = 0;
   size_t pack_src_ct = 0;
   size_t pack_out = 0;
-  size_t pack_row = 0;
-  size_t v1_row1 = 0;
   size_t v1_shift_src = 0;
   size_t v1_rot_dst = 0, v1_rot_a = 0, v1_rot_b = 0;
   size_t v1_sum_dst = 0, v1_sum_a = 0, v1_sum_b = 0;
```

Result: no change. 89.44 queries/s (-0.5%).
